# ArmingLou/seed-vc

Measured on AMD Instinct MI355X. Metric: mel_frames_per_sec, higher is better.
Workload: dtype f16; 1 GPU; seed-uvit-tat-xlsr-tiny CFM 25 steps cfg 0.7 + HiFT, batch 64 x (P=430,S=430) per GPU; batch_per_gpu=64, global_batch=64, prompt_frames=430, diffusion_steps=25, vocoder_precision=fp16p8, lanes_per_gpu=2, parallelism=utterance-sharded x1, audio gather on rank 0

## Files before the change

### include/seedvc_hip.h

```cpp
#ifndef SEEDVC_HIP_H
#define SEEDVC_HIP_H

#include <stdint.h>

#ifdef __cplusplus
extern "C" {
#endif

#define SVC_ABI_VERSION 1

typedef struct svc_tensor_desc {
    const char* name;
    const float* data;
    int ndim;
    int64_t shape[4];
} svc_tensor_desc_t;

typedef struct svc_dit_config {
    int version;
    int hidden_dim, num_heads, depth, in_channels, content_dim, style_dim;
    int final_layer_type;
    int time_as_token, style_as_token, uvit_skip_connection, long_skip_connection, style_condition;
    int wn_hidden_dim, wn_num_layers, wn_kernel_size, wn_dilation_rate;
} svc_dit_config_t;

typedef struct svc_dit svc_dit_t;

int svc_dit_create(const svc_dit_config_t* cfg, const svc_tensor_desc_t* weights, int n_weights,
                   void* stream, svc_dit_t** out);
void svc_dit_destroy(svc_dit_t* m);

int svc_dit_set_microbatch(svc_dit_t* m, int utterances);

int svc_dit_set_fused_min_rows(svc_dit_t* m, long rows);
int svc_dit_fused_available(svc_dit_t* m);
int svc_dit_set_graphs(svc_dit_t* m, int on);

typedef struct svc_cfm_args {
    int B;
    int T;
    int P;
    const float* mu;
    const float* prompt;
    const float* style;
    const float* z;
    const int64_t* x_lens;
    const int64_t* prompt_lens;
    int n_timesteps;
    float temperature;
    float cfg_rate[2];
    int random_voice;
    float* out;
} svc_cfm_args_t;

int svc_cfm_sample(svc_dit_t* m, const svc_cfm_args_t* args, void* stream);

int svc_dit_forward(svc_dit_t* m, int N, int T, const float* x, const float* prompt_x, const int64_t* x_lens,
                    float t, const float* style, const float* mu, float* out, void* stream);

typedef struct svc_bigvgan_config {
    int num_mels, upsample_initial_channel, num_upsamples, num_kernels;
    int upsample_rates[8], upsample_kernel_sizes[8];
    int resblock_kernel_sizes[4], resblock_dilation_sizes[4][3];
    int use_tanh_at_final, use_bias_at_final, snake_logscale, snakebeta;
    int precision;
} svc_bigvgan_config_t;
typedef struct svc_bigvgan svc_bigvgan_t;
int svc_bigvgan_create(const svc_bigvgan_config_t* cfg, const svc_tensor_desc_t* weights, int n_weights,
                       void* stream, svc_bigvgan_t** out);
void svc_bigvgan_destroy(svc_bigvgan_t* m);
int svc_bigvgan_forward(svc_bigvgan_t* m, const float* mel, int B, int S, float* out, void* stream);
int svc_bigvgan_forward_ragged(svc_bigvgan_t* m, const float* mel, const int32_t* lens, int B, int S, float* out, void* stream);

typedef struct svc_hift_config {
    int in_channels, base_channels, nb_harmonics, sampling_rate;
    float nsf_alpha, nsf_sigma, nsf_voiced_threshold;
    int num_upsamples, upsample_rates[4], upsample_kernel_sizes[4];
    int istft_n_fft, istft_hop;
    int num_kernels, resblock_kernel_sizes[4], resblock_dilation_sizes[4][3];
    int source_resblock_kernel_sizes[4], source_resblock_dilation_sizes[4][3];
    float lrelu_slope, audio_limit;
    int f0_cond_channels;
    int precision;
} svc_hift_config_t;
typedef struct svc_hift svc_hift_t;
int svc_hift_create(const svc_hift_config_t* cfg, const svc_tensor_desc_t* weights, int n_weights,
                    void* stream, svc_hift_t** out);
void svc_hift_destroy(svc_hift_t* m);
int svc_hift_forward(svc_hift_t* m, const float* mel, const float* f0, const float* phase0, const float* noise,
                     int B, int S, float* out, float* f0_out, void* stream);
int svc_hift_forward_ragged(svc_hift_t* m, const float* mel, const int32_t* lens, const float* f0, const float* phase0,
                            const float* noise, int B, int S, float* out, float* f0_out, void* stream);
int svc_bigvgan_set_microbatch(svc_bigvgan_t* m, int utterances);
int svc_hift_set_microbatch(svc_hift_t* m, int utterances);

typedef struct svc_ar_config {
    int dim, n_head, n_local_heads, head_dim, n_layer, intermediate_size, vocab_size, max_seq_len;
    float rope_base, norm_eps;
} svc_ar_config_t;
typedef struct svc_ar svc_ar_t;
int svc_ar_create(const svc_ar_config_t* cfg, const svc_tensor_desc_t* weights, int n_weights, void* stream, svc_ar_t** out);
void svc_ar_destroy(svc_ar_t* m);
int svc_ar_reset(svc_ar_t* m, void* stream);
int svc_ar_forward_generate(svc_ar_t* m, const float* x, int S, const int64_t* input_pos, const int64_t* kv_pos,
                            float* logits_out, void* stream);
int svc_ar_decode_step(svc_ar_t* m, const float* x, int set_pos, int64_t input_pos, int64_t kv_pos, float* logits_out,
                       void* stream);
int svc_ar_generate(svc_ar_t* m, const float* x_prefill, int S, const int64_t* input_pos, const int64_t* kv_pos,
                    const float* exp_noise, int max_new, int min_tokens_before_eos, float temperature, float top_p,
                    float repetition_penalty, int check_every, int32_t* tokens_out, int32_t* n_tokens, void* stream);
int svc_ar_set_max_batch(svc_ar_t* m, int max_batch, void* stream);
int svc_ar_prefill_slot(svc_ar_t* m, int slot, const float* x, int S, const int64_t* input_pos, const int64_t* kv_pos,
                        float* logits_out, void* stream);
int svc_ar_decode_step_batch(svc_ar_t* m, int B, const float* x, int set_pos, const int64_t* input_pos, const int64_t* kv_pos,
                             float* logits_out, void* stream);
int svc_ar_generate_batch(svc_ar_t* m, int B, const float* x_prefill, const int32_t* S, const int64_t* input_pos,
                          const int64_t* kv_pos, const float* exp_noise, int max_new, int min_tokens_before_eos, float temperature,
                          float top_p, float repetition_penalty, int check_every, int32_t* tokens_out, int32_t* n_tokens,
                          void* stream);
int svc_ar_generate_batch_seeded(svc_ar_t* m, int B, const float* x_prefill, const int32_t* S, const int64_t* input_pos,
                                 const int64_t* kv_pos, const uint64_t* seeds, int max_new, int min_tokens_before_eos,
                                 float temperature, float top_p, float repetition_penalty, int check_every, int32_t* tokens_out,
                                 int32_t* n_tokens, void* stream);
int svc_ar_exp_draws(svc_ar_t* m, uint64_t seed, int step0, int n_steps, float* out, void* stream);
int svc_ar_prefill_batch(svc_ar_t* m, int n, const int32_t* slots, const float* x, const int32_t* S, const int64_t* input_pos,
                         const int64_t* kv_pos, float* logits_out, void* stream);
int svc_ar_set_prefill_rows(svc_ar_t* m, int rows);
int svc_ar_prefill_passes(svc_ar_t* m);
typedef struct svc_ar_request {
    int32_t slot;
    int32_t S;
    const float* exp_noise;
    uint64_t seed;
    int32_t max_new;
    int32_t min_tokens_before_eos;
    float temperature, top_p, repetition_penalty;
    int32_t* tokens_out;
} svc_ar_request_t;
int svc_ar_admit(svc_ar_t* m, int n, const svc_ar_request_t* requests, const float* x_prefill, const int64_t* input_pos,
                 const int64_t* kv_pos, void* stream);
int svc_ar_run(svc_ar_t* m, int n_steps, int32_t* n_tokens, int32_t* done, void* stream);
int svc_ar_retire(svc_ar_t* m, int slot, void* stream);
int svc_ar_session_active(svc_ar_t* m);
int svc_ar_sample(svc_ar_t* m, const float* logits, const int32_t* prev_tokens, int n_prev, int suppress_token,
                  float temperature, float top_p, float repetition_penalty, const float* exp_noise, int32_t* idx_out,
                  float* probs_out, void* stream);

typedef struct svc_lr_config {
    int channels, in_channels, out_channels;
    int is_discrete, codebook_size;
    int n_convs;
    int interpolate;
    int has_final_conv;
    int f0_condition, n_f0_bins;
} svc_lr_config_t;
typedef struct svc_lr svc_lr_t;
int svc_lr_create(const svc_lr_config_t* cfg, const svc_tensor_desc_t* weights, int n_weights, void* stream, svc_lr_t** out);
void svc_lr_destroy(svc_lr_t* m);
int svc_lr_forward(svc_lr_t* m, const float* x, const int64_t* tokens, const int32_t* in_lens, int B, int tin_max,
                   const int32_t* ylens, int tout_max, const float* f0, const int32_t* f0_lens, int tf0_max, float* out,
                   void* stream);

int svc_v2_assemble_cond(const float* prompt_cond, const int32_t* prompt_lens, const float* cond, const int32_t* cond_lens, int B,
                         int Pmax, int Smax, int Dc, int T, float* out, void* stream);
int svc_mel_strip_prompt(const float* mel, const int32_t* prompt_lens, const int32_t* x_lens, int B, int C, int T, int Smax,
                         float pad_value, float* out, void* stream);

int svc_anti_alias_act_fwd(const void* x, void* y, const float* up12, const float* down12,
                           const float* log_alpha, const float* log_beta, int B, int C, int L, int dtype,
                           void* stream);

typedef struct svc_mel svc_mel_t;
int svc_mel_create(int n_fft, int hop, int win, int n_mels, const float* window, const float* mel_basis, void* stream,
                   svc_mel_t** out);
void svc_mel_destroy(svc_mel_t* m);
int svc_mel_frames(const svc_mel_t* m, int L);
int svc_mel_forward(svc_mel_t* m, const float* y, int B, int L, float* out, void* stream);

typedef struct svc_campplus_config {
    int feat_dim, embedding_size, growth_rate, bn_size, init_channels, m_channels;
    int n_blocks, block_layers[4], block_kernel[4], block_dilation[4];
    int seg_len;
} svc_campplus_config_t;
typedef struct svc_campplus svc_campplus_t;
int svc_campplus_create(const svc_campplus_config_t* cfg, const svc_tensor_desc_t* weights, int n_weights, void* stream,
                        svc_campplus_t** out);
void svc_campplus_destroy(svc_campplus_t* m);
int svc_campplus_forward(svc_campplus_t* m, const float* feat, int B, int T, float* out, void* stream);
int svc_kaldi_fbank_frames(int n_samples);
int svc_kaldi_fbank(svc_campplus_t* m, const float* wave, int n_samples, float* out, void* stream);

int svc_crossfade(float* chunk2, const float* chunk1_tail, const double* fade_in, const double* fade_out, int n,
                  void* stream);

int svc_chunks_gather_cond(const float* prompt_cond, const int32_t* prompt_lens, int U, int Pmax, const float* cond, int R,
                           const int32_t* utt, const int32_t* row0, const int32_t* rows, int N, int Dc, int T, float* mu,
                           void* stream);
int svc_chunks_assemble(const float* wave, long long stride, const int32_t* lens, const int32_t* first, const int32_t* last, int N,
                        const double* fade_in, const double* fade_out, int ov, float* out, long long out_len, void* stream);

int svc_sola_step(const float* wave, long long stride, int start, int N, float* sola_state, int max_slots, const int32_t* slots,
                  const float* fade_in, const float* fade_out, int block, int Lb, int Ls, float* out, int32_t* offsets,
                  void* stream);

int svc_op_linear(const float* a, const float* w, const float* bias, float* c, int M, int N, int K, int dtype,
                  int act, void* stream);
int svc_op_conv1d(const float* x, const float* w, const float* bias, float* y, int B, int L, int Cin, int Cout,
                  int k, int dilation, int stride, int pad_left, int Lout, int pad_mode, int dtype, void* stream);
typedef struct {
    const float* x; const uint16_t* a_hi; const uint16_t* a_lo;
    const float* w; const float* bias;
    int32_t B, L, Cin, Cout, k, dilation, pad_left, Lout, dtype;
    const int32_t* seq_len;
    const float* res; const float* res2;
    float out_scale; int32_t act; float act_slope;
    int32_t c_rows, c_off;
    const float* post_a; const float* post_ib; int32_t next_p8;
    int32_t bm, force_gemm;
    float* y; uint16_t* plane_hi; uint16_t* plane_lo;
    int32_t took;
} svc_conv1d_ex_t;
int svc_op_conv1d_ex(svc_conv1d_ex_t* args, void* stream);
int svc_op_conv1d_last_took(void);
int svc_op_conv_transpose1d(const float* x, const float* w, const float* bias, float* y, int B, int L, int Cin,
                            int Cout, int k, int stride, int dtype, void* stream);
int svc_op_attention(const float* q, const float* k, const float* v, float* out, int N, int T, int H,
                     const int64_t* kv_lens_host, void* stream);
int svc_op_rmsnorm(const float* x, const float* gamma, const float* w, const float* b, int add_one, float* y,
                   int rows, int D, void* stream);

int svc_op_gemm_bench(int M, int N, int K, int dtype, int epi, int iters, int debug, float* out_ms, void* stream);
int svc_op_gemm_forms_diff(int M, int N, int K, int epi, int debug_a, int debug_b, long long* n_diff, void* stream);

int svc_prof_enable(int on);
int svc_prof_collect(double* out, int n_cls);

const char* svc_last_error(void);
int svc_abi_version(void);

#ifdef __cplusplus
}
#endif
#endif
```

### seed-vc_amd/_lib.py

```python
import ctypes as C
import os

import torch

_HERE = os.path.dirname(os.path.abspath(__file__))
LIB_PATH = os.path.join(_HERE, "libseedvc_hip.so")

EXPORTS = [
    "svc_abi_version", "svc_last_error",
    "svc_dit_create", "svc_dit_destroy", "svc_dit_set_microbatch", "svc_dit_set_fused_min_rows", "svc_dit_fused_available", "svc_dit_set_graphs", "svc_cfm_sample", "svc_dit_forward",
    "svc_bigvgan_create", "svc_bigvgan_destroy", "svc_bigvgan_forward", "svc_bigvgan_forward_ragged", "svc_bigvgan_set_microbatch",
    "svc_hift_create", "svc_hift_destroy", "svc_hift_forward", "svc_hift_forward_ragged", "svc_hift_set_microbatch",
    "svc_anti_alias_act_fwd",
    "svc_ar_create", "svc_ar_destroy", "svc_ar_reset", "svc_ar_forward_generate", "svc_ar_decode_step", "svc_ar_sample", "svc_ar_generate",
    "svc_ar_set_max_batch", "svc_ar_prefill_slot", "svc_ar_decode_step_batch", "svc_ar_generate_batch",
    "svc_ar_generate_batch_seeded", "svc_ar_exp_draws", "svc_v2_assemble_cond", "svc_mel_strip_prompt",
    "svc_ar_prefill_batch", "svc_ar_set_prefill_rows", "svc_ar_prefill_passes", "svc_ar_admit", "svc_ar_run", "svc_ar_retire",
    "svc_ar_session_active",
    "svc_lr_create", "svc_lr_destroy", "svc_lr_forward", "svc_crossfade",
    "svc_chunks_gather_cond", "svc_chunks_assemble", "svc_sola_step",
    "svc_campplus_create", "svc_campplus_destroy", "svc_campplus_forward", "svc_kaldi_fbank_frames", "svc_kaldi_fbank",
    "svc_mel_create", "svc_mel_destroy", "svc_mel_frames", "svc_mel_forward",
    "svc_prof_enable", "svc_prof_collect",
    "svc_op_linear", "svc_op_conv1d", "svc_op_conv1d_ex", "svc_op_conv1d_last_took", "svc_op_conv_transpose1d", "svc_op_attention", "svc_op_rmsnorm",
]


class TensorDesc(C.Structure):
    _fields_ = [("name", C.c_char_p), ("data", C.c_void_p), ("ndim", C.c_int), ("shape", C.c_int64 * 4)]


class DitConfig(C.Structure):
    _fields_ = [(n, C.c_int) for n in (
        "version", "hidden_dim", "num_heads", "depth", "in_channels", "content_dim", "style_dim",
        "final_layer_type", "time_as_token", "style_as_token", "uvit_skip_connection", "long_skip_connection",
        "style_condition", "wn_hidden_dim", "wn_num_layers", "wn_kernel_size", "wn_dilation_rate")]


class CfmArgs(C.Structure):
    _fields_ = [("B", C.c_int), ("T", C.c_int), ("P", C.c_int),
                ("mu", C.c_void_p), ("prompt", C.c_void_p), ("style", C.c_void_p), ("z", C.c_void_p),
                ("x_lens", C.POINTER(C.c_int64)), ("prompt_lens", C.POINTER(C.c_int64)),
                ("n_timesteps", C.c_int), ("temperature", C.c_float), ("cfg_rate", C.c_float * 2),
                ("random_voice", C.c_int), ("out", C.c_void_p)]


class BigVGANConfig(C.Structure):
    _fields_ = [("num_mels", C.c_int), ("upsample_initial_channel", C.c_int), ("num_upsamples", C.c_int),
                ("num_kernels", C.c_int), ("upsample_rates", C.c_int * 8), ("upsample_kernel_sizes", C.c_int * 8),
                ("resblock_kernel_sizes", C.c_int * 4), ("resblock_dilation_sizes", (C.c_int * 3) * 4),
                ("use_tanh_at_final", C.c_int), ("use_bias_at_final", C.c_int), ("snake_logscale", C.c_int),
                ("snakebeta", C.c_int), ("precision", C.c_int)]


class HiftConfig(C.Structure):
    _fields_ = [("in_channels", C.c_int), ("base_channels", C.c_int), ("nb_harmonics", C.c_int),
                ("sampling_rate", C.c_int), ("nsf_alpha", C.c_float), ("nsf_sigma", C.c_float),
                ("nsf_voiced_threshold", C.c_float), ("num_upsamples", C.c_int), ("upsample_rates", C.c_int * 4),
                ("upsample_kernel_sizes", C.c_int * 4), ("istft_n_fft", C.c_int), ("istft_hop", C.c_int),
                ("num_kernels", C.c_int), ("resblock_kernel_sizes", C.c_int * 4),
                ("resblock_dilation_sizes", (C.c_int * 3) * 4), ("source_resblock_kernel_sizes", C.c_int * 4),
                ("source_resblock_dilation_sizes", (C.c_int * 3) * 4), ("lrelu_slope", C.c_float),
                ("audio_limit", C.c_float), ("f0_cond_channels", C.c_int), ("precision", C.c_int)]


class ArConfig(C.Structure):
    _fields_ = [(n, C.c_int) for n in ("dim", "n_head", "n_local_heads", "head_dim", "n_layer", "intermediate_size",
                                       "vocab_size", "max_seq_len")] + [("rope_base", C.c_float), ("norm_eps", C.c_float)]


class ArRequest(C.Structure):
    _fields_ = [("slot", C.c_int32), ("S", C.c_int32), ("exp_noise", C.c_void_p), ("seed", C.c_uint64), ("max_new", C.c_int32),
                ("min_tokens_before_eos", C.c_int32), ("temperature", C.c_float), ("top_p", C.c_float),
                ("repetition_penalty", C.c_float), ("tokens_out", C.c_void_p)]


class CampplusConfig(C.Structure):
    _fields_ = [(n, C.c_int) for n in ("feat_dim", "embedding_size", "growth_rate", "bn_size", "init_channels", "m_channels", "n_blocks")] + \
               [("block_layers", C.c_int * 4), ("block_kernel", C.c_int * 4), ("block_dilation", C.c_int * 4), ("seg_len", C.c_int)]


class LrConfig(C.Structure):
    _fields_ = [(n, C.c_int) for n in ("channels", "in_channels", "out_channels", "is_discrete", "codebook_size", "n_convs",
                                       "interpolate", "has_final_conv", "f0_condition", "n_f0_bins")]


class Conv1dEx(C.Structure):
    _fields_ = [("x", C.c_void_p), ("a_hi", C.c_void_p), ("a_lo", C.c_void_p), ("w", C.c_void_p), ("bias", C.c_void_p)] + \
               [(n, C.c_int32) for n in ("B", "L", "Cin", "Cout", "k", "dilation", "pad_left", "Lout", "dtype")] + \
               [("seq_len", C.POINTER(C.c_int32)), ("res", C.c_void_p), ("res2", C.c_void_p),
                ("out_scale", C.c_float), ("act", C.c_int32), ("act_slope", C.c_float), ("c_rows", C.c_int32), ("c_off", C.c_int32),
                ("post_a", C.c_void_p), ("post_ib", C.c_void_p), ("next_p8", C.c_int32), ("bm", C.c_int32), ("force_gemm", C.c_int32),
                ("y", C.c_void_p), ("plane_hi", C.c_void_p), ("plane_lo", C.c_void_p), ("took", C.c_int32)]


_lib = None


def lib():
    global _lib
    if _lib is None:
        if not os.path.exists(LIB_PATH):
            raise ImportError(f"{LIB_PATH} is missing: run `python -c 'import __graft_entry__ as g; g.build()'` "
                              f"(hipcc --offload-arch=gfx950); there is no CPU fallback")
        l = C.CDLL(LIB_PATH)
        l.svc_last_error.restype = C.c_char_p
        if l.svc_abi_version() != 1:
            raise ImportError("libseedvc_hip.so ABI version mismatch")
        l.svc_sola_step.argtypes = [C.c_void_p, C.c_longlong, C.c_int, C.c_int, C.c_void_p, C.c_int, C.POINTER(C.c_int32),
                                    C.c_void_p, C.c_void_p, C.c_int, C.c_int, C.c_int, C.c_void_p, C.c_void_p, C.c_void_p]
        l.svc_hift_forward_ragged.argtypes = [C.c_void_p, C.c_void_p, C.POINTER(C.c_int32), C.c_void_p, C.c_void_p, C.c_void_p,
                                              C.c_int, C.c_int, C.c_void_p, C.c_void_p, C.c_void_p]
        l.svc_op_conv1d_ex.argtypes = [C.POINTER(Conv1dEx), C.c_void_p]
        _lib = l
    return _lib


def check(rc):
    if rc != 0:
        raise RuntimeError("seedvc_hip: " + (lib().svc_last_error() or b"unknown error").decode())


def stream_ptr():
    return C.c_void_p(torch.cuda.current_stream().cuda_stream)


def ptr(t):
    return C.c_void_p(t.data_ptr()) if t is not None else C.c_void_p(0)


def f32c(t, device=None):
    t = t.detach()
    if device is not None:
        t = t.to(device)
    return t.to(torch.float32).contiguous()


def make_descs(state_dict, device):
    keep, items = [], []
    for k, v in state_dict.items():
        if not torch.is_tensor(v) or not (v.is_floating_point()):
            continue
        if v.dim() > 4:
            continue
        t = f32c(v, device)
        keep.append(t)
        items.append((k, t))
    arr = (TensorDesc * len(items))()
    for i, (k, t) in enumerate(items):
        kb = k.encode()
        keep.append(kb)
        arr[i].name = kb
        arr[i].data = t.data_ptr()
        arr[i].ndim = t.dim()
        for j in range(4):
            arr[i].shape[j] = t.shape[j] if j < t.dim() else 1
    return arr, len(items), keep


def i64_host(values):
    if values is None:
        return None
    vals = [int(v) for v in values]
    return (C.c_int64 * len(vals))(*vals)
```

### seed-vc_amd/cfm.py

```python
import ctypes as C

import torch

from . import _lib
from .specs import dit_config


def _cfg_struct(cfg):
    c = _lib.DitConfig()
    c.version = cfg["version"]
    c.hidden_dim, c.num_heads, c.depth = cfg["D"], cfg["H"], cfg["L"]
    c.in_channels, c.content_dim, c.style_dim = cfg["C"], cfg["Dc"], cfg["style_dim"]
    c.final_layer_type = 1 if cfg["head"] == "wavenet" else 0
    c.time_as_token, c.style_as_token = int(cfg["time_as_token"]), int(cfg["style_as_token"])
    c.uvit_skip_connection, c.long_skip_connection = int(cfg["uvit"]), int(cfg["long_skip"])
    c.style_condition = int(cfg["style_condition"])
    c.wn_hidden_dim = cfg.get("wn_dim", 0)
    c.wn_num_layers = cfg.get("wn_layers", 0)
    c.wn_kernel_size = cfg.get("wn_kernel", 0)
    c.wn_dilation_rate = cfg.get("wn_dilation", 1)
    return c


class Estimator:

    def __init__(self, cfg, state_dict, device="cuda:0"):
        self.cfg = cfg
        self.device = torch.device(device)
        self.in_channels = cfg["C"]
        self._h = C.c_void_p()
        with torch.cuda.device(self.device):
            descs, n, keep = _lib.make_descs(state_dict, self.device)
            cs = _cfg_struct(cfg)
            _lib.check(_lib.lib().svc_dit_create(C.byref(cs), descs, n, _lib.stream_ptr(), C.byref(self._h)))
            torch.cuda.current_stream().synchronize()
        del keep

    def setup_caches(self, max_batch_size=1, max_seq_length=8192):
        return None

    def set_microbatch(self, n):
        _lib.check(_lib.lib().svc_dit_set_microbatch(self._h, int(n)))

    def set_fused_min_rows(self, rows):
        _lib.check(_lib.lib().svc_dit_set_fused_min_rows(self._h, C.c_long(int(rows))))

    def set_graphs(self, on):
        _lib.check(_lib.lib().svc_dit_set_graphs(self._h, int(bool(on))))

    @property
    def fused_available(self):
        return bool(_lib.lib().svc_dit_fused_available(self._h))

    def __call__(self, x, prompt_x, x_lens, t, style, cond, mask_content=False):
        N, Cc, T = x.shape
        with torch.cuda.device(self.device):
            x, prompt_x, style, cond = (_lib.f32c(a, self.device) for a in (x, prompt_x, style, cond))
            out = torch.empty_like(x)
            tval = float(t.reshape(-1)[0]) if torch.is_tensor(t) else float(t)
            lens = None
            if x_lens is not None:
                xl = [int(v) for v in (x_lens.tolist() if torch.is_tensor(x_lens) else x_lens)]
                if len(xl) == 1 and N > 1:
                    xl = xl * N
                lens = _lib.i64_host(xl)
            _lib.check(_lib.lib().svc_dit_forward(self._h, N, T, _lib.ptr(x), _lib.ptr(prompt_x), lens,
                                                  C.c_float(tval), _lib.ptr(style), _lib.ptr(cond), _lib.ptr(out),
                                                  _lib.stream_ptr()))
        return out

    def close(self):
        if self._h:
            _lib.lib().svc_dit_destroy(self._h)
            self._h = C.c_void_p()

    def __del__(self):
        try:
            self.close()
        except Exception:
            pass


class CFM:

    def __init__(self, cfg, state_dict, device="cuda:0"):
        self.cfg = cfg
        self.estimator = Estimator(cfg, state_dict, device)
        self.in_channels = cfg["C"]
        self.device = self.estimator.device

    @classmethod
    def from_preset(cls, name, state_dict, device="cuda:0", **overrides):
        return cls(dit_config(name, **overrides), state_dict, device)

    @torch.inference_mode()
    def inference(self, mu, x_lens, prompt, style, f0=None, n_timesteps=10, temperature=1.0,
                  inference_cfg_rate=0.5, random_voice=False, z=None, prompt_lens=None):
        if self.cfg["version"] == 2 and not isinstance(f0, (type(None), torch.Tensor)):
            n_timesteps, f0 = f0, None
        B, T = mu.size(0), mu.size(1)
        dev = self.device
        with torch.cuda.device(dev):
            mu, prompt, style = (_lib.f32c(a, dev) for a in (mu, prompt, style))
            if z is None:
                z = torch.randn([B, self.in_channels, T], device=dev)
            z = _lib.f32c(z, dev)
            out = torch.empty(B, self.in_channels, T, device=dev, dtype=torch.float32)
            a = _lib.CfmArgs()
            a.B, a.T, a.P = B, T, prompt.size(-1)
            a.mu, a.prompt, a.style, a.z, a.out = (t.data_ptr() for t in (mu, prompt, style, z, out))
            xl = None
            if x_lens is not None:
                xl = [int(v) for v in (x_lens.tolist() if torch.is_tensor(x_lens) else x_lens)]
                if len(xl) == 1 and B > 1:
                    xl = xl * B
            lens_keep = _lib.i64_host(xl)
            plens_keep = _lib.i64_host(prompt_lens)
            a.x_lens = lens_keep
            a.prompt_lens = plens_keep
            a.n_timesteps = int(n_timesteps)
            a.temperature = float(temperature)
            if isinstance(inference_cfg_rate, (list, tuple)):
                a.cfg_rate[0], a.cfg_rate[1] = float(inference_cfg_rate[0]), float(inference_cfg_rate[1])
            else:
                a.cfg_rate[0], a.cfg_rate[1] = float(inference_cfg_rate), float(inference_cfg_rate)
            a.random_voice = int(bool(random_voice))
            _lib.check(_lib.lib().svc_cfm_sample(self.estimator._h, C.byref(a), _lib.stream_ptr()))
        return out
```

### seed-vc_amd/csrc/common.h

```cpp
#pragma once
#include <atomic>
#include <hip/hip_runtime.h>
#include <stdint.h>
#include <stdio.h>
#include <string>

namespace svc {

typedef _Float16 half_t;
typedef _Float16 half8 __attribute__((ext_vector_type(8)));
typedef _Float16 half4 __attribute__((ext_vector_type(4)));
typedef _Float16 half2v __attribute__((ext_vector_type(2)));
typedef float float4v __attribute__((ext_vector_type(4)));
typedef unsigned int u32x4 __attribute__((ext_vector_type(4)));

void set_error(const std::string& msg);
const char* get_error();

#define SVC_CHECK_HIP(expr)                                                                  \
    do {                                                                                     \
        hipError_t _e = (expr);                                                              \
        if (_e != hipSuccess) {                                                              \
            svc::set_error(std::string(#expr) + ": " + hipGetErrorString(_e) + " at " + __FILE__ + \
                           ":" + std::to_string(__LINE__));                                  \
            return 1;                                                                        \
        }                                                                                    \
    } while (0)

#define SVC_REQUIRE(cond, msg)                                                               \
    do {                                                                                     \
        if (!(cond)) {                                                                       \
            svc::set_error(std::string("requirement failed: ") + #cond + " -- " + (msg));    \
            return 1;                                                                        \
        }                                                                                    \
    } while (0)

__device__ __forceinline__ float sin_sq(float x) {
    const float n = rintf(x * 0.318309886183790672f);
    float r = fmaf(n, -3.140625f, x);
    r = fmaf(n, -9.67502593994140625e-4f, r);
    r = fmaf(n, -1.509957990978376e-7f, r);
    const float r2 = r * r;
    float p = fmaf(r2, 2.6348154733568663e-06f, -0.00019822761532850564f);
    p = fmaf(p, r2, 0.008333242498338223f);
    p = fmaf(p, r2, -0.1666666567325592f);
    const float sn = fmaf(p * r2, r, r);
    return sn * sn;
}

struct DeviceState {
    int device = -1;
    void* zero_page = nullptr;
    std::atomic<unsigned long long> kconv_attr{0};
    std::atomic<bool> fused_attr{false};
};
DeviceState* device_state();
int current_device();

enum { PROF_KGEMM_F16 = 0, PROF_KGEMM_F32 = 1, PROF_ATTN = 2, PROF_FUSED = 3, PROF_N = 4 };
bool prof_enabled();
void prof_begin(int cls, hipStream_t st);
void prof_end(int cls, double flops, double bytes, hipStream_t st, unsigned long long tag = 0);

template <int MAXA, int DPT>
__device__ __forceinline__ void wait_tiles(int ahead) {
    static_assert(MAXA * DPT <= 63, "vmcnt is a 6-bit counter");
    if constexpr (MAXA <= 0) {
        asm volatile("s_waitcnt vmcnt(0)" ::: "memory");
    } else {
        if (ahead >= MAXA) asm volatile("s_waitcnt vmcnt(%0)" ::"n"(MAXA * DPT) : "memory");
        else wait_tiles<MAXA - 1, DPT>(ahead);
    }
}

__device__ __forceinline__ float act_apply(float v, int act, float slope);
__device__ __forceinline__ uint4 pack8(const float* v) {
    half8 h;
#pragma unroll
    for (int j = 0; j < 8; ++j) h[j] = (half_t)v[j];
    return *reinterpret_cast<uint4*>(&h);
}

static inline int cdiv(long a, long b) { return (int)((a + b - 1) / b); }
static inline long round_up(long a, long b) { return (a + b - 1) / b * b; }

constexpr int KG_MAX_TAPS = 48;

enum { KG_PAD_ZERO = 0, KG_PAD_REFLECT = 1, KG_PAD_CLAMP = 2 };
enum { KG_ACT_NONE = 0, KG_ACT_SILU = 1, KG_ACT_ELU = 2, KG_ACT_LRELU = 3, KG_ACT_TANH = 4, KG_ACT_ABS = 5,
       KG_ACT_CLAMP = 6 , KG_ACT_SIGMOID = 7 };
enum {
    KG_EPI_STORE = 0,
    KG_EPI_SWIGLU = 1,
    KG_EPI_TANHSIG = 2,
    KG_EPI_QKV_ROPE = 3,
};

__device__ __forceinline__ float act_apply(float v, int act, float slope) {
    switch (act) {
        case KG_ACT_SILU: return v / (1.0f + __expf(-v));
        case KG_ACT_ELU: return v > 0.f ? v : (expm1f(v));
        case KG_ACT_LRELU: return v > 0.f ? v : v * slope;
        case KG_ACT_TANH: return tanhf(v);
        case KG_ACT_ABS: return fabsf(v);
        case KG_ACT_CLAMP: return fminf(fmaxf(v, -slope), slope);
        case KG_ACT_SIGMOID: return 1.0f / (1.0f + __expf(-v));
        default: return v;
    }
}

struct KGemmParams {
    const void* a_ptr[KG_MAX_TAPS];
    long a_ld[KG_MAX_TAPS];
    int a_shift[KG_MAX_TAPS];
    int a_ktiles[KG_MAX_TAPS];
    int n_taps;
    int Lout, a_seq_rows, a_off, a_stride, a_len, pad_mode;
    int reflect_min;
    const int* seq_len;
    const void* zero_page;
    float prof_flop_scale;
    int debug;
    int group_n;
    const void* w;
    long ldw;
    int M, N;
    int c_seq_rows, c_off;
    float* c32; long ldc32;
    half_t* c16; long ldc16;
    const float* post_a; const float* post_ib; int post_n; half_t* c16_lo;
    const float* bias;
    const float* rowvec; long ld_rowvec;
    const float* gate;   long ld_gate;
    const float* res;    long ldres;
    const float* res2;   long ldres2;
    float out_scale;
    int act; float act_slope;
    int post_relu;
    int vec_ok;
    const float* rope;
    int rope_D;
    float q_scale;
    half_t* vt; long vt_seq_stride; long vt_ld;
    int vt_mode;
};

int kgemm_launch(const KGemmParams& p, int dtype , int epi, hipStream_t st);
int kgemm_big_launch(const KGemmParams& p, int epi, hipStream_t st);

struct KConvParams {
    const void* a_hi; const void* a_lo;
    const void* w; long ldw;
    const float* bias;
    int B, Lin, Lout, N, cin_pad, k, dil, pad_left, nsub;
    int c_seq_rows, c_off;
    float* c32; long ldc32;
    half_t* c16; half_t* c16_lo; long ldc16;
    const float* post_a; const float* post_ib; int post_n;
    const float* res; long ldres;
    const float* res2; long ldres2;
    float out_scale;
    int act; float act_slope;
    const void* zero_page;
    int w8_exp;
    int c16_lo_fmt;
    const int* seq_len;
    int bm;
    int* took;
};
bool kconv_enabled();
int kconv_launch(const KConvParams& p, hipStream_t st);
__device__ __forceinline__ unsigned lo_pair_p8(float hi_as_float, float lo) {
    const float a = __builtin_amdgcn_fmed3f(hi_as_float, -448.f, 448.f), b = __builtin_amdgcn_fmed3f(lo * 2048.f, -448.f, 448.f);
    return (unsigned)__builtin_amdgcn_cvt_pk_fp8_f32(a, b, 0, false) & 0xffffu;
}
int kconv_pack_p8(const float* src, unsigned short* dst, int n0, int n1, int n2, long s0, long s1, long s2, long d0, long d1, long d2,
                  const float* scale, int* exp_out, hipStream_t st);

struct PanelParams {
    int M;
    int Lout, seq_rows, row_off;
    const half_t* wstream;
    int n_slots;
    float eps;
    int do_post;
    const half_t* ao;
    float* x;
    const float* gate_a; const float* gate_f;
    const float* g_ffn; const float* w_f; const float* b_f; int add_one;
    int I;
    half_t* c16;
    int do_skip;
    const half_t* skip_in; const float* bskip;
    int do_qkv;
    const float* g_attn; const float* w_a; const float* b_a;
    const float* rope; float q_scale;
    half_t* qk; half_t* vt; long vt_seq_stride; long vt_ld; int vt_mode;
    int do_final;
    const float* g_fin; const float* w_fin; const float* b_fin; half_t* n16;
};
bool fused_supported(int D, int I);
long fused_stream_halfs(int D, int I, bool post, bool skip, bool qkv);
long fused_pack_stream(half_t* dst, int D, int I, const float* wo, const float* w1, const float* w3, const float* w2,
                       const float* wskip, const float* wqkv, hipStream_t st);
int fused_panel_launch(const PanelParams& p, int D, bool gated, hipStream_t st);

struct AttnParams {
    const half_t* q; const half_t* k; long ld_qk;
    const half_t* vt; long vt_seq_stride; long vt_ld;
    half_t* out; long ld_out;
    int n_seq, H, seq_rows, Tq;
    int q_start;
    const int* kv_len; int kv_len_const;
    int vt_perm;
};
__host__ __device__ inline int vt_perm_pos(int pos) {
    return (pos & ~31) | (((pos >> 2) & 3) << 3) | (((pos >> 4) & 1) << 2) | (pos & 3);
}
__host__ __device__ inline int vt_perm_pos16(int pos) {
    return (pos & ~12) | ((pos & 4) << 1) | ((pos & 8) >> 1);
}
__host__ __device__ inline int vt_pos(int pos, int mode) {
    return mode == 2 ? vt_perm_pos16(pos) : (mode == 1 ? vt_perm_pos(pos) : pos);
}
int attention_vt_mode(int n_seq, int H, int Tq);
int attention_launch(const AttnParams& p, hipStream_t st);
int attention_permute_vt(half_t* vt, long rows, long vt_ld, int mode, hipStream_t st);

int rmsnorm_mod_launch(const float* x, long ldx, half_t* y, long ldy, const float* gamma,
                       const float* w, const float* b, long ld_wb, int add_one,
                       int rows, int D, int seq_rows, float eps, hipStream_t st);
int layernorm_mod_launch(const float* x, long ldx, half_t* y, long ldy, const float* scale,
                         const float* shift, int rows, int D, float eps, hipStream_t st);

}
```

### seed-vc_amd/csrc/device.hip

```cpp
#include <map>
#include <mutex>

#include "common.h"

namespace svc {

int current_device() {
    int d = -1;
    if (hipGetDevice(&d) != hipSuccess) return -1;
    return d;
}

DeviceState* device_state() {
    static std::mutex mu;
    static std::map<int, DeviceState*> states;
    const int d = current_device();
    if (d < 0) {
        set_error("hipGetDevice failed");
        return nullptr;
    }
    std::lock_guard<std::mutex> lk(mu);
    auto it = states.find(d);
    if (it != states.end()) return it->second;
    void* zp = nullptr;
    if (hipMalloc(&zp, 256) != hipSuccess || hipMemset(zp, 0, 256) != hipSuccess) {
        set_error("device_state: zero page allocation failed");
        return nullptr;
    }
    DeviceState* s = new DeviceState();
    s->device = d;
    s->zero_page = zp;
    states[d] = s;
    return s;
}

}
```

### seed-vc_amd/csrc/dit.hip

```cpp
#include <math.h>
#include <string.h>

#include <algorithm>
#include <vector>

#include "model_util.h"

using namespace svc;

namespace {
constexpr int MAX_STREAMS = 3;
constexpr int ROPE_POS = 8192;

float bf16_round(float f) {
    uint32_t u;
    memcpy(&u, &f, 4);
    u = (u + 0x7FFF + ((u >> 16) & 1)) & 0xFFFF0000u;
    memcpy(&f, &u, 4);
    return f;
}

std::vector<float> linspace01(int n) {
    std::vector<float> v(n);
    const float step = 1.0f / (float)(n - 1);
    const int half = n / 2;
    for (int i = 0; i < n; ++i) v[i] = i < half ? 0.0f + step * (float)i : 1.0f - step * (float)(n - 1 - i);
    return v;
}
}

struct svc_dit {
    svc_dit_config_t cfg;
    int D, H, L, C, Dc, S, I, W, NL, WK, npre, C16, C32;
    bool v2, wavenet, adaptive_blocks;
    Arena wts, ws;
    struct StepGraph {
        std::vector<float> key;
        hipGraphExec_t exec = nullptr;
        int seen = 0;
    };
    std::vector<StepGraph> graphs;
    hipStream_t cap_stream = nullptr;
    int use_graphs = 0;
    void drop_graphs() {
        for (auto& g : graphs) if (g.exec) (void)hipGraphExecDestroy(g.exec);
        graphs.clear();
    }
    PinnedRing staging;
    hipStream_t create_stream;
    int device = -1;

    struct Layer {
        half_t *wqkv, *wo, *w13, *w2, *wskip;
        float *bskip, *g_attn, *g_ffn;
        half_t* stream = nullptr;
        int stream_slots = 0;
    };
    half_t* stream_pre = nullptr;
    int stream_pre_slots = 0;
    bool fused_ok = false;
    long fused_min_rows = 10240;
    std::vector<Layer> layers;
    float* g_final;
    std::vector<int> emit, recv;
    float *te_w0, *te_b0, *te_w2, *te_b2, *te_freqs;
    float *te2_w0, *te2_b0, *te2_w2, *te2_b2, *te2_freqs;
    float *mod_w, *mod_b;
    int mod_n;
    int mod_layer_n;
    half_t* w_merge_x;
    float* w_stat;
    float* stat_const;
    float* w_style_merge;
    float *style_in_w, *style_in_b;
    half_t *head_wa, *head_w2;
    float *head_b0, *head_b2;
    half_t *w_longskip, *w_conv1, *w_resproj, *w_fl, *w_conv2;
    float *b_longskip, *b_conv1, *b_resproj, *b_fl, *b_conv2;
    float *wn_cond_w, *wn_cond_b, *fl_mod_w, *fl_mod_b;
    std::vector<half_t*> wn_in, wn_res, wn_skip;
    std::vector<float*> wn_res_b, wn_skip_b;
    half_t* wn_tail = nullptr;
    float* b_tail = nullptr;
    long acts_stride = 0;
    float* rope;

    int cap_streams = 0, cap_B = 0, cap_T = 0, cap_steps = 0;
    int seq_rows = 0, vt_ld = 0;
    float *x32, *xin, *st_term, *v32, *u_rowvec, *tok_style, *prompt32, *wnx32, *flin32;
    half_t *x16, *n16, *qk16, *vt, *ao16, *ff16, *h16, *hm16, *xr16, *wnx16, *acts16, *fl16, *fo16;
    std::vector<half_t*> skip16;
    int *d_kvlen, *d_convlen, *d_plen;
    int* d_convlen_w = nullptr;
    int win0 = 0;
    float *d_tvals, *d_tfeat, *d_th, *d_t1, *d_t1s, *d_t2, *d_mod, *d_gcond, *d_flmod, *d_stylevec;
    int microbatch = 0;

    int pack(const StateDict& sd, hipStream_t st);
    int reserve(int n_streams, int B, int T, int n_steps, hipStream_t st);
    int tables(const std::vector<float>& tvals, hipStream_t st);
    int statics(int n_streams, const int (*flags)[3], int B, int T, const float* mu, const float* style_dev,
                hipStream_t st);
    int run_group(const svc_cfm_args_t* a, int b0, int nb, int n_streams, const int (*flags)[3],
                  const std::vector<float>& tvals, const std::vector<float>& dts, float c0, float ca, float cb,
                  int stream_a, int stream_b, hipStream_t st);
    int body(int n_streams, int B, int T, int step, hipStream_t st);
    int body_fused(int n_streams, int B, int T, int step, hipStream_t st);
    int head(int n_streams, int B, int T, int step, hipStream_t st);
};

namespace {

int pack_block(int dtype, const float* src, long src_ld, long src_col, int N, int K, void* dst, long ldw, long dst_col,
               long dst_row0, long dst_row_step, const float* scale, hipStream_t st) {
    return pack_any(dtype, src + src_col, dst, dst_row0 * ldw + dst_col, N, 1, K, src_ld, 0, 1, dst_row_step * ldw, 0, 1,
                    scale, st);
}

float* copy_vec(Arena& ar, const float* src, long n, hipStream_t st) {
    float* d = ar.alloc_n<float>(n, st);
    if (!d) return nullptr;
    if (hipMemcpyAsync(d, src, n * sizeof(float), hipMemcpyDeviceToDevice, st) != hipSuccess) {
        set_error("hipMemcpyAsync failed");
        return nullptr;
    }
    return d;
}

}

#define GETW(var, name, ...)                                              \
    const svc_tensor_desc_t* var = sd.get(name);                          \
    if (require_shape(var, name, {__VA_ARGS__})) return 1;

int svc_dit::pack(const StateDict& sd, hipStream_t st) {
    const long Dp = round_up(D, 128);
    auto new16 = [&](long rows, long ld) { return wts.alloc_n<half_t>(round_up(rows, 128) * ld, st); };
    layers.resize(L);
    for (int i = 0; i < L; ++i) {
        const std::string p = "transformer.layers." + std::to_string(i) + ".";
        Layer& ly = layers[i];
        GETW(wqkv, p + "attention.wqkv.weight", 3 * D, D);
        GETW(wo, p + "attention.wo.weight", D, D);
        GETW(w1, p + "feed_forward.w1.weight", I, D);
        GETW(w3, p + "feed_forward.w3.weight", I, D);
        GETW(w2, p + "feed_forward.w2.weight", D, I);
        ly.wqkv = new16(3 * D, D);
        ly.wo = new16(D, D);
        ly.w13 = new16(2 * I, D);
        ly.w2 = new16(D, I);
        if (!ly.wqkv || !ly.wo || !ly.w13 || !ly.w2) return 1;
        if (pack_block(0, wqkv->data, D, 0, 3 * D, D, ly.wqkv, D, 0, 0, 1, nullptr, st)) return 1;
        if (pack_block(0, wo->data, D, 0, D, D, ly.wo, D, 0, 0, 1, nullptr, st)) return 1;
        if (pack_block(0, w1->data, D, 0, I, D, ly.w13, D, 0, 0, 2, nullptr, st)) return 1;
        if (pack_block(0, w3->data, D, 0, I, D, ly.w13, D, 0, 1, 2, nullptr, st)) return 1;
        if (pack_block(0, w2->data, I, 0, D, I, ly.w2, I, 0, 0, 1, nullptr, st)) return 1;
        const std::string an = v2 ? p + "attention_norm.norm.weight" : p + "attention_norm.norm.weight";
        const std::string fn = v2 ? p + "ffn_norm.weight" : p + "ffn_norm.norm.weight";
        GETW(ga, an, D);
        GETW(gf, fn, D);
        ly.g_attn = copy_vec(wts, ga->data, D, st);
        ly.g_ffn = copy_vec(wts, gf->data, D, st);
        if (!ly.g_attn || !ly.g_ffn) return 1;
        ly.wskip = nullptr;
        ly.bskip = nullptr;
        if (std::find(recv.begin(), recv.end(), i) != recv.end()) {
            GETW(ws_, p + "skip_in_linear.weight", D, 2 * D);
            GETW(bs_, p + "skip_in_linear.bias", D);
            ly.wskip = new16(D, 2 * D);
            if (!ly.wskip) return 1;
            if (pack_block(0, ws_->data, 2 * D, 0, D, 2 * D, ly.wskip, 2 * D, 0, 0, 1, nullptr, st)) return 1;
            ly.bskip = copy_vec(wts, bs_->data, D, st);
            if (!ly.bskip) return 1;
        }
    }
    {
        GETW(gn, "transformer.norm.norm.weight", D);
        g_final = copy_vec(wts, gn->data, D, st);
        if (!g_final) return 1;
    }
    fused_ok = fused_supported(D, I);
    if (fused_ok) {
        auto W = [&](const std::string& k) { return sd.get(k)->data; };
        const int slot_halfs = (D / 16) * 512;
        for (int i = 0; i < L; ++i) {
            const std::string p = "transformer.layers." + std::to_string(i) + ".";
            const bool last = i == L - 1;
            const bool nskip = !last && layers[i + 1].wskip != nullptr;
            const std::string pn = "transformer.layers." + std::to_string(i + 1) + ".";
            const long halfs = fused_stream_halfs(D, I, true, nskip, !last);
            layers[i].stream = wts.alloc_n<half_t>(halfs, st);
            if (!layers[i].stream) return 1;
            const long wr = fused_pack_stream(layers[i].stream, D, I, W(p + "attention.wo.weight"), W(p + "feed_forward.w1.weight"),
                                              W(p + "feed_forward.w3.weight"), W(p + "feed_forward.w2.weight"),
                                              nskip ? W(pn + "skip_in_linear.weight") : nullptr,
                                              last ? nullptr : W(pn + "attention.wqkv.weight"), st);
            if (wr != halfs) { set_error("fused stream packing failed"); return 1; }
            layers[i].stream_slots = (int)(halfs / slot_halfs);
        }
        const long halfs = fused_stream_halfs(D, I, false, false, true);
        stream_pre = wts.alloc_n<half_t>(halfs, st);
        if (!stream_pre) return 1;
        if (fused_pack_stream(stream_pre, D, I, nullptr, nullptr, nullptr, nullptr, nullptr,
                              W("transformer.layers.0.attention.wqkv.weight"), st) != halfs) { set_error("fused stream packing failed"); return 1; }
        stream_pre_slots = (int)(halfs / slot_halfs);
    }
    mod_layer_n = adaptive_blocks ? (v2 ? 6 * D : 4 * D) : 0;
    mod_n = L * mod_layer_n + 2 * D;
    mod_w = wts.alloc_n<float>((long)mod_n * D, st);
    mod_b = wts.alloc_n<float>(mod_n, st);
    if (!mod_w || !mod_b) return 1;
    auto put_mod = [&](const std::string& wname, const std::string& bname, int rows, long row0) -> int {
        GETW(w, wname, rows, D);
        GETW(b, bname, rows);
        if (pack_f32_launch(w->data, mod_w + row0 * D, rows, 1, D, D, 0, 1, D, 0, 1, nullptr, st)) return 1;
        SVC_CHECK_HIP(hipMemcpyAsync(mod_b + row0, b->data, rows * sizeof(float), hipMemcpyDeviceToDevice, st));
        return 0;
    };
    for (int i = 0; i < L && adaptive_blocks; ++i) {
        const std::string p = "transformer.layers." + std::to_string(i) + ".";
        if (v2) {
            if (put_mod(p + "attention_norm.linear.weight", p + "attention_norm.linear.bias", 6 * D, (long)i * mod_layer_n)) return 1;
        } else {
            if (put_mod(p + "attention_norm.project_layer.weight", p + "attention_norm.project_layer.bias", 2 * D, (long)i * mod_layer_n)) return 1;
            if (put_mod(p + "ffn_norm.project_layer.weight", p + "ffn_norm.project_layer.bias", 2 * D, (long)i * mod_layer_n + 2 * D)) return 1;
        }
    }
    if (v2) {
        if (put_mod("transformer.norm.linear.weight", "transformer.norm.linear.bias", 2 * D, (long)L * mod_layer_n)) return 1;
    } else {
        if (put_mod("transformer.norm.project_layer.weight", "transformer.norm.project_layer.bias", 2 * D, (long)L * mod_layer_n)) return 1;
    }
    auto put_temb = [&](const std::string& p, int dim, float** w0, float** b0, float** w2, float** b2, float** fr) -> int {
        GETW(a, p + ".mlp.0.weight", dim, 256);
        GETW(b, p + ".mlp.0.bias", dim);
        GETW(c, p + ".mlp.2.weight", dim, dim);
        GETW(d, p + ".mlp.2.bias", dim);
        *w0 = copy_vec(wts, a->data, (long)dim * 256, st);
        *b0 = copy_vec(wts, b->data, dim, st);
        *w2 = copy_vec(wts, c->data, (long)dim * dim, st);
        *b2 = copy_vec(wts, d->data, dim, st);
        if (!*w0 || !*b0 || !*w2 || !*b2) return 1;
        if (const auto* f = sd.get(p + ".freqs")) {
            if (require_shape(f, p + ".freqs", {128})) return 1;
            *fr = copy_vec(wts, f->data, 128, st);
        } else {
            std::vector<float> h(128);
            for (int i = 0; i < 128; ++i) h[i] = expf(-logf(10000.0f) * (float)i / 128.0f);
            *fr = wts.alloc_n<float>(128, st);
            if (*fr) SVC_CHECK_HIP(hipMemcpyAsync(*fr, h.data(), 512, hipMemcpyHostToDevice, st));
            SVC_CHECK_HIP(hipStreamSynchronize(st));
        }
        return *fr ? 0 : 1;
    };
    if (put_temb("t_embedder", D, &te_w0, &te_b0, &te_w2, &te_b2, &te_freqs)) return 1;

    const bool style_in_merge = !v2 && cfg.style_condition && !cfg.style_as_token;
    const int Kin = D + 2 * C + (style_in_merge ? S : 0);
    GETW(wm, "cond_x_merge_linear.weight", D, Kin);
    GETW(bm, "cond_x_merge_linear.bias", D);
    GETW(wcp, "cond_projection.weight", D, Dc);
    GETW(bcp, "cond_projection.bias", D);
    w_merge_x = new16(D, C16);
    if (!w_merge_x) return 1;
    if (pack_block(0, wm->data, Kin, 0, D, C, w_merge_x, C16, 0, 0, 1, nullptr, st)) return 1;
    const long Ks = C32 + Dc;
    w_stat = wts.alloc_n<float>(Dp * Ks, st);
    stat_const = wts.alloc_n<float>(D, st);
    if (!w_stat || !stat_const) return 1;
    if (pack_block(1, wm->data, Kin, C, D, C, w_stat, Ks, 0, 0, 1, nullptr, st)) return 1;
    {
        float* wcpT = ws.alloc_n<float>((long)Dc * D, st);
        if (!wcpT) return 1;
        if (pack_f32_launch(wcp->data, wcpT, D, 1, Dc, Dc, 0, 1, 1, 0, D, nullptr, st)) return 1;
        if (small_linear_launch(wm->data + 2 * C, Kin, wcpT, D, nullptr, w_stat + C32, Ks, D, Dc, D, KG_ACT_NONE, st)) return 1;
        if (small_linear_launch(bcp->data, D, wm->data + 2 * C, Kin, bm->data, stat_const, D, 1, D, D, KG_ACT_NONE, st)) return 1;
    }
    w_style_merge = nullptr;
    if (style_in_merge) {
        w_style_merge = wts.alloc_n<float>((long)D * S, st);
        if (!w_style_merge) return 1;
        if (pack_f32_launch(wm->data + 2 * C + D, w_style_merge, D, 1, S, Kin, 0, 1, S, 0, 1, nullptr, st)) return 1;
    }
    style_in_w = style_in_b = nullptr;
    if (v2 || cfg.style_as_token) {
        GETW(sw, "style_in.weight", D, S);
        GETW(sb, "style_in.bias", D);
        style_in_w = copy_vec(wts, sw->data, (long)D * S, st);
        style_in_b = copy_vec(wts, sb->data, D, st);
        if (!style_in_w || !style_in_b) return 1;
    }
    if (!wavenet) {
        GETW(a, "final_mlp.0.weight", D, D);
        GETW(b, "final_mlp.0.bias", D);
        GETW(c, "final_mlp.2.weight", C, D);
        GETW(d, "final_mlp.2.bias", C);
        head_wa = new16(D, D);
        head_w2 = new16(C, D);
        if (!head_wa || !head_w2) return 1;
        if (pack_block(0, a->data, D, 0, D, D, head_wa, D, 0, 0, 1, nullptr, st)) return 1;
        if (pack_block(0, c->data, D, 0, C, D, head_w2, D, 0, 0, 1, nullptr, st)) return 1;
        head_b0 = copy_vec(wts, b->data, D, st);
        head_b2 = copy_vec(wts, d->data, C, st);
        if (!head_b0 || !head_b2) return 1;
    } else {
        if (put_temb("t_embedder2", W, &te2_w0, &te2_b0, &te2_w2, &te2_b2, &te2_freqs)) return 1;
        if (cfg.long_skip_connection) {
            GETW(a, "skip_linear.weight", D, D + C);
            GETW(b, "skip_linear.bias", D);
            w_longskip = new16(D, D + C16);
            if (!w_longskip) return 1;
            if (pack_block(0, a->data, D + C, 0, D, D + C, w_longskip, D + C16, 0, 0, 1, nullptr, st)) return 1;
            b_longskip = copy_vec(wts, b->data, D, st);
            if (!b_longskip) return 1;
        }
        GETW(c1w, "conv1.weight", W, D);
        GETW(c1b, "conv1.bias", W);
        GETW(rpw, "res_projection.weight", W, D);
        GETW(rpb, "res_projection.bias", W);
        GETW(c2w, "conv2.weight", C, W, 1);
        GETW(c2b, "conv2.bias", C);
        w_conv1 = new16(W, D);
        w_resproj = new16(W, D);
        w_conv2 = new16(C, W);
        if (!w_conv1 || !w_resproj || !w_conv2) return 1;
        if (pack_block(0, c1w->data, D, 0, W, D, w_conv1, D, 0, 0, 1, nullptr, st)) return 1;
        if (pack_block(0, rpw->data, D, 0, W, D, w_resproj, D, 0, 0, 1, nullptr, st)) return 1;
        if (pack_block(0, c2w->data, W, 0, C, W, w_conv2, W, 0, 0, 1, nullptr, st)) return 1;
        b_conv1 = copy_vec(wts, c1b->data, W, st);
        b_resproj = copy_vec(wts, rpb->data, W, st);
        b_conv2 = copy_vec(wts, c2b->data, C, st);
        if (!b_conv1 || !b_resproj || !b_conv2) return 1;
        {
            WeightSrc fl;
            if (resolve_weight(sd, "final_layer.linear", wts, st, &fl)) return 1;
            if (require_shape(fl.desc, "final_layer.linear.weight", {W, W})) return 1;
            GETW(flb, "final_layer.linear.bias", W);
            GETW(mw, "final_layer.adaLN_modulation.1.weight", 2 * W, W);
            GETW(mb, "final_layer.adaLN_modulation.1.bias", 2 * W);
            w_fl = new16(W, W);
            if (!w_fl) return 1;
            if (pack_block(0, fl.v, W, 0, W, W, w_fl, W, 0, 0, 1, fl.scale, st)) return 1;
            b_fl = copy_vec(wts, flb->data, W, st);
            fl_mod_w = copy_vec(wts, mw->data, 2L * W * W, st);
            fl_mod_b = copy_vec(wts, mb->data, 2 * W, st);
            if (!b_fl || !fl_mod_w || !fl_mod_b) return 1;
        }
        {
            WeightSrc cl;
            if (resolve_weight(sd, "wavenet.cond_layer.conv.conv", wts, st, &cl)) return 1;
            if (require_shape(cl.desc, "wavenet.cond_layer.conv.conv.weight", {2L * W * NL, W, 1})) return 1;
            GETW(clb, "wavenet.cond_layer.conv.conv.bias", 2L * W * NL);
            wn_cond_w = wts.alloc_n<float>(2L * W * NL * W, st);
            wn_cond_b = wts.alloc_n<float>(2L * W * NL, st);
            float* tmp_b = ws.alloc_n<float>(2L * W * NL, st);
            if (!wn_cond_w || !wn_cond_b || !tmp_b) return 1;
            wn_in.resize(NL);
            wn_res.assign(NL, nullptr);
            wn_skip.resize(NL);
            wn_res_b.assign(NL, nullptr);
            wn_skip_b.resize(NL);
            for (int i = 0; i < NL; ++i) {
                const std::string li = std::to_string(i);
                for (int half = 0; half < 2; ++half) {
                    const long src_row0 = 2L * W * i + (long)half * W;
                    if (pack_f32_launch(cl.v + src_row0 * W, wn_cond_w + (2L * W * i + half) * W, W, 1, W, W, 0, 1, 2L * W, 0, 1,
                                        cl.scale ? cl.scale + src_row0 : nullptr, st)) return 1;
                    if (pack_f32_launch(clb->data + src_row0, tmp_b + 2L * W * i + half, W, 1, 1, 1, 0, 0, 2, 0, 0, nullptr, st)) return 1;
                }
                WeightSrc in;
                if (resolve_weight(sd, "wavenet.in_layers." + li + ".conv.conv", wts, st, &in)) return 1;
                if (require_shape(in.desc, "wavenet.in_layers." + li + ".conv.conv.weight", {2L * W, W, WK})) return 1;
                GETW(inb, "wavenet.in_layers." + li + ".conv.conv.bias", 2L * W);
                wn_in[i] = new16(2 * W, (long)WK * W);
                float* inb_perm = ws.alloc_n<float>(2L * W, st);
                if (!wn_in[i] || !inb_perm) return 1;
                for (int half = 0; half < 2; ++half) {
                    if (pack_f16_launch(in.v + (long)half * W * W * WK, wn_in[i] + (long)half * WK * W, W, WK, W,
                                        (long)W * WK, 1, WK, 2L * WK * W, W, 1, in.scale ? in.scale + (long)half * W : nullptr, st)) return 1;
                    if (pack_f32_launch(inb->data + (long)half * W, inb_perm + half, W, 1, 1, 1, 0, 0, 2, 0, 0, nullptr, st)) return 1;
                }
                {
                    float* dst = wn_cond_b + 2L * W * i;
                    if (add_rowvec_launch(dst, tmp_b + 2L * W * i, 0, inb_perm, 1, 2 * W, st)) return 1;
                }
                WeightSrc rs;
                const int rs_out = i < NL - 1 ? 2 * W : W;
                if (resolve_weight(sd, "wavenet.res_skip_layers." + li + ".conv.conv", wts, st, &rs)) return 1;
                if (require_shape(rs.desc, "wavenet.res_skip_layers." + li + ".conv.conv.weight", {rs_out, W, 1})) return 1;
                GETW(rsb, "wavenet.res_skip_layers." + li + ".conv.conv.bias", rs_out);
                const long skip_row0 = i < NL - 1 ? W : 0;
                if (i < NL - 1) {
                    wn_res[i] = new16(W, W);
                    if (!wn_res[i]) return 1;
                    if (pack_block(0, rs.v, W, 0, W, W, wn_res[i], W, 0, 0, 1, rs.scale, st)) return 1;
                    wn_res_b[i] = copy_vec(wts, rsb->data, W, st);
                    if (!wn_res_b[i]) return 1;
                }
                wn_skip[i] = new16(W, W);
                if (!wn_skip[i]) return 1;
                if (pack_block(0, rs.v + skip_row0 * W, W, 0, W, W, wn_skip[i], W, 0, 0, 1,
                               rs.scale ? rs.scale + skip_row0 : nullptr, st)) return 1;
                wn_skip_b[i] = copy_vec(wts, rsb->data + skip_row0, W, st);
                if (!wn_skip_b[i]) return 1;
            }
        }
    }
    if (wavenet) {
        const long Kt = (long)NL * W + D;
        wn_tail = new16(W, Kt);
        b_tail = wts.alloc_n<float>(W, st);
        if (!wn_tail || !b_tail) return 1;
        for (int i = 0; i < NL; ++i)
            SVC_CHECK_HIP(hipMemcpy2DAsync(wn_tail + (long)i * W, Kt * 2, wn_skip[i], (size_t)W * 2, (size_t)W * 2, W, hipMemcpyDeviceToDevice, st));
        SVC_CHECK_HIP(hipMemcpy2DAsync(wn_tail + (long)NL * W, Kt * 2, w_resproj, (size_t)D * 2, (size_t)D * 2, W, hipMemcpyDeviceToDevice, st));
        if (add_rowvec_launch(b_tail, b_resproj, 0, wn_skip_b[0], 1, W, st)) return 1;
        for (int i = 1; i < NL; ++i)
            if (add_rowvec_launch(b_tail, b_tail, 0, wn_skip_b[i], 1, W, st)) return 1;
    }
    {
        std::vector<float> tab((size_t)ROPE_POS * 32 * 2);
        for (int i = 0; i < 32; ++i) {
            const float e = (float)(2 * i) / 64.0f;
            const float f = 1.0f / powf(10000.0f, e);
            for (int t = 0; t < ROPE_POS; ++t) {
                const float a = (float)t * f;
                float c = (float)cos((double)a), s = (float)sin((double)a);
                if (v2) { c = bf16_round(c); s = bf16_round(s); }
                tab[((size_t)t * 32 + i) * 2] = c;
                tab[((size_t)t * 32 + i) * 2 + 1] = s;
            }
        }
        rope = wts.alloc_n<float>(tab.size(), st);
        if (!rope) return 1;
        SVC_CHECK_HIP(hipMemcpyAsync(rope, tab.data(), tab.size() * 4, hipMemcpyHostToDevice, st));
        SVC_CHECK_HIP(hipStreamSynchronize(st));
    }
    SVC_CHECK_HIP(hipStreamSynchronize(st));
    ws.release();
    return 0;
}

int svc_dit::reserve(int n_streams, int B, int T, int n_steps, hipStream_t st) {
    if (n_streams <= cap_streams && B <= cap_B && T <= cap_T && n_steps <= cap_steps) {
        seq_rows = (int)round_up(T + npre, 8);
        vt_ld = (int)round_up(seq_rows, 64);
        return 0;
    }
    SVC_CHECK_HIP(hipStreamSynchronize(st));
    drop_graphs();
    ws.release();
    cap_streams = std::max(cap_streams, n_streams);
    cap_B = std::max(cap_B, B);
    cap_T = std::max(cap_T, T);
    cap_steps = std::max(cap_steps, n_steps);
    const long rows_seq = round_up(cap_T + npre, 8);
    const long nseq = (long)cap_streams * cap_B;
    const long M = nseq * rows_seq;
    const long vtl = round_up(rows_seq, 64);
    x32 = ws.alloc_n<float>((long)cap_B * rows_seq * C16, st);
    x16 = ws.alloc_n<half_t>(M * C16, st);
    xin = ws.alloc_n<float>(M * D, st);
    st_term = ws.alloc_n<float>(M * D, st);
    v32 = ws.alloc_n<float>(M * C16, st);
    u_rowvec = ws.alloc_n<float>(nseq * D, st);
    tok_style = ws.alloc_n<float>(nseq * D, st);
    prompt32 = ws.alloc_n<float>((long)cap_B * rows_seq * C32, st);
    n16 = ws.alloc_n<half_t>(M * D, st);
    qk16 = ws.alloc_n<half_t>(M * 2 * D, st);
    vt = ws.alloc_n<half_t>(nseq * D * vtl, st);
    ao16 = ws.alloc_n<half_t>(M * D, st);
    ff16 = ws.alloc_n<half_t>(M * I, st);
    h16 = ws.alloc_n<half_t>(M * D, st);
    skip16.assign(emit.size(), nullptr);
    for (auto& p : skip16) {
        p = ws.alloc_n<half_t>(M * D, st);
        if (!p) return 1;
    }
    if (!x32 || !x16 || !xin || !st_term || !v32 || !u_rowvec || !tok_style || !prompt32 || !n16 || !qk16 || !vt ||
        !ao16 || !ff16 || !h16)
        return 1;
    hm16 = xr16 = wnx16 = acts16 = fl16 = fo16 = nullptr;
    wnx32 = flin32 = nullptr;
    if (!wavenet) {
        hm16 = ws.alloc_n<half_t>(M * D, st);
        if (!hm16) return 1;
    } else {
        xr16 = ws.alloc_n<half_t>(M * D, st);
        wnx32 = ws.alloc_n<float>(M * W, st);
        wnx16 = ws.alloc_n<half_t>(M * W, st);
        acts_stride = M * W;
        acts16 = ws.alloc_n<half_t>((long)NL * acts_stride, st);
        flin32 = ws.alloc_n<float>(M * W, st);
        fl16 = ws.alloc_n<half_t>(M * W, st);
        fo16 = ws.alloc_n<half_t>(M * W, st);
        if (!xr16 || !wnx32 || !wnx16 || !acts16 || !flin32 || !fl16 || !fo16) return 1;
    }
    d_kvlen = ws.alloc_n<int>(nseq, st);
    d_convlen = ws.alloc_n<int>(nseq, st);
    d_convlen_w = ws.alloc_n<int>(nseq, st);
    d_plen = ws.alloc_n<int>(cap_B, st);
    const long Sx = cap_steps;
    d_tvals = ws.alloc_n<float>(Sx, st);
    d_tfeat = ws.alloc_n<float>(Sx * 256, st);
    d_th = ws.alloc_n<float>(Sx * std::max(D, W), st);
    d_t1 = ws.alloc_n<float>(Sx * D, st);
    d_t1s = ws.alloc_n<float>(Sx * D, st);
    d_t2 = ws.alloc_n<float>(Sx * std::max(W, 1), st);
    d_mod = ws.alloc_n<float>(Sx * mod_n, st);
    d_gcond = ws.alloc_n<float>(Sx * std::max(2L * W * NL, 1L), st);
    d_flmod = ws.alloc_n<float>(Sx * std::max(2 * W, 1), st);
    d_stylevec = ws.alloc_n<float>((long)cap_B * D, st);
    if (!d_kvlen || !d_convlen || !d_convlen_w || !d_plen || !d_tvals || !d_tfeat || !d_th || !d_t1 || !d_t1s || !d_t2 || !d_mod ||
        !d_gcond || !d_flmod || !d_stylevec)
        return 1;
    seq_rows = (int)round_up(T + npre, 8);
    vt_ld = (int)round_up(seq_rows, 64);
    SVC_CHECK_HIP(hipStreamSynchronize(st));
    return 0;
}

int svc_dit::tables(const std::vector<float>& tvals, hipStream_t st) {
    const int n = (int)tvals.size();
    {
        float* h = reinterpret_cast<float*>(staging.acquire(n * sizeof(float)));
        if (!h) return 1;
        memcpy(h, tvals.data(), n * sizeof(float));
        SVC_CHECK_HIP(hipMemcpyAsync(d_tvals, h, n * sizeof(float), hipMemcpyHostToDevice, st));
        if (staging.commit(st)) return 1;
    }
    if (timestep_feat_launch(d_tvals, te_freqs, d_tfeat, n, st)) return 1;
    if (small_linear_launch(d_tfeat, 256, te_w0, 256, te_b0, d_th, D, n, D, 256, KG_ACT_SILU, st)) return 1;
    if (small_linear_launch(d_th, D, te_w2, D, te_b2, d_t1, D, n, D, D, KG_ACT_NONE, st)) return 1;
    if (silu_launch(d_t1, d_t1s, (long)n * D, st)) return 1;
    if (small_linear_launch(v2 ? d_t1s : d_t1, D, mod_w, D, mod_b, d_mod, mod_n, n, mod_n, D, KG_ACT_NONE, st)) return 1;
    if (wavenet) {
        if (small_linear_launch(d_tfeat, 256, te2_w0, 256, te2_b0, d_th, W, n, W, 256, KG_ACT_SILU, st)) return 1;
        if (small_linear_launch(d_th, W, te2_w2, W, te2_b2, d_t2, W, n, W, W, KG_ACT_NONE, st)) return 1;
        if (small_linear_launch(d_t2, W, wn_cond_w, W, wn_cond_b, d_gcond, 2L * W * NL, n, 2 * W * NL, W, KG_ACT_NONE, st)) return 1;
        if (small_linear_launch(d_t1s, D, fl_mod_w, W, fl_mod_b, d_flmod, 2 * W, n, 2 * W, W, KG_ACT_NONE, st)) return 1;
    }
    return 0;
}


namespace {
KGemmParams gemm_base(int M, int N, int Lout) {
    KGemmParams p;
    memset(&p, 0, sizeof(p));
    p.M = M;
    p.N = N;
    p.Lout = Lout;
    p.a_seq_rows = Lout;
    p.c_seq_rows = Lout;
    p.a_stride = 1;
    p.a_len = Lout;
    p.n_taps = 1;
    p.vec_ok = 1;
    return p;
}
}

int svc_dit::body(int n_streams, int B, int T, int step, hipStream_t st) {
    const int nseq = n_streams * B;
    const int M = nseq * seq_rows;
    const float* mod = d_mod + (long)step * mod_n;
    if (prefix_rows_launch(xin, nseq, seq_rows, D, npre, T + npre, d_t1 + (long)step * D, tok_style,
                           cfg.time_as_token ? 1 : 0, st)) return 1;
    {
        KGemmParams p = gemm_base(nseq * T, D, T);
        p.a_ptr[0] = x16; p.a_ld[0] = C16; p.a_ktiles[0] = C16 / 64;
        p.a_seq_rows = seq_rows; p.a_len = T;
        p.w = w_merge_x; p.ldw = C16;
        p.c_seq_rows = seq_rows; p.c_off = npre;
        p.c32 = xin; p.ldc32 = D;
        p.res = st_term; p.ldres = D;
        if (kgemm_launch(p, 0, KG_EPI_STORE, st)) return 1;
    }
    if (fused_ok && (long)M >= fused_min_rows) {
        if (body_fused(n_streams, B, T, step, st)) return 1;
        return head(n_streams, B, T, step, st);
    }
    const int Lw = seq_rows - win0;
    auto gemm_win = [&](int N) {
        KGemmParams p = gemm_base(nseq * Lw, N, Lw);
        p.a_seq_rows = seq_rows; p.c_seq_rows = seq_rows;
        p.a_off = win0; p.c_off = win0;
        return p;
    };
    size_t emit_i = 0;
    std::vector<int> skip_stack;
    for (int i = 0; i < L; ++i) {
        const bool tail_only = i == L - 1 && win0 > 0;

        const Layer& ly = layers[i];
        const float* lmod = adaptive_blocks ? mod + (long)i * mod_layer_n : nullptr;
        const bool is_recv = ly.wskip != nullptr;
        if (is_recv) {
            const int src = skip_stack.back();
            skip_stack.pop_back();
            KGemmParams p = gemm_base(M, D, seq_rows);
            p.n_taps = 2;
            p.a_ptr[0] = h16; p.a_ld[0] = D; p.a_ktiles[0] = D / 64;
            p.a_ptr[1] = skip16[src]; p.a_ld[1] = D; p.a_ktiles[1] = D / 64;
            p.w = ly.wskip; p.ldw = 2 * D;
            p.bias = ly.bskip;
            p.c32 = xin; p.ldc32 = D;
            if (kgemm_launch(p, 0, KG_EPI_STORE, st)) return 1;
        }
        const float *w_a = nullptr, *b_a = nullptr, *gate_a = nullptr, *w_f = nullptr, *b_f = nullptr, *gate_f = nullptr;
        if (lmod) {
            if (v2) {
                b_a = lmod; w_a = lmod + D; gate_a = lmod + 2 * D;
                b_f = lmod + 3 * D; w_f = lmod + 4 * D; gate_f = lmod + 5 * D;
            } else {
                w_a = lmod; b_a = lmod + D; w_f = lmod + 2 * D; b_f = lmod + 3 * D;
            }
        }
        if (rmsnorm_mod_launch(xin, D, n16, D, ly.g_attn, w_a, b_a, 0, v2 ? 1 : 0, M, D, seq_rows, 1e-5f, st)) return 1;
        {
            KGemmParams p = gemm_base(M, 3 * D, seq_rows);
            p.a_ptr[0] = n16; p.a_ld[0] = D; p.a_ktiles[0] = D / 64;
            p.w = ly.wqkv; p.ldw = D;
            p.c16 = qk16; p.ldc16 = 2 * D;
            p.rope = rope; p.rope_D = D; p.q_scale = 0.125f * 1.4426950408889634f;
            p.vt = vt; p.vt_seq_stride = (long)D * vt_ld; p.vt_ld = vt_ld; p.vt_mode = attention_vt_mode(nseq, H, seq_rows);
            if (kgemm_launch(p, 0, KG_EPI_QKV_ROPE, st)) return 1;
        }
        {
            AttnParams a;
            memset(&a, 0, sizeof(a));
            a.q = qk16; a.k = qk16 + D; a.ld_qk = 2 * D;
            a.vt = vt; a.vt_seq_stride = (long)D * vt_ld; a.vt_ld = vt_ld; a.vt_perm = attention_vt_mode(nseq, H, seq_rows);
            a.out = ao16; a.ld_out = D;
            a.n_seq = nseq; a.H = H; a.seq_rows = seq_rows; a.Tq = seq_rows;
            a.q_start = tail_only ? win0 : 0;
            a.kv_len = d_kvlen;
            if (attention_launch(a, st)) return 1;
        }
        {
            KGemmParams p = tail_only ? gemm_win(D) : gemm_base(M, D, seq_rows);
            p.a_ptr[0] = ao16; p.a_ld[0] = D; p.a_ktiles[0] = D / 64;
            p.w = ly.wo; p.ldw = D;
            p.gate = gate_a; p.ld_gate = 0;
            p.res = xin; p.ldres = D;
            p.c32 = xin; p.ldc32 = D;
            if (kgemm_launch(p, 0, KG_EPI_STORE, st)) return 1;
        }
        if (rmsnorm_mod_launch(xin, D, n16, D, ly.g_ffn, w_f, b_f, 0, v2 ? 1 : 0, M, D, seq_rows, 1e-5f, st)) return 1;
        {
            KGemmParams p = tail_only ? gemm_win(2 * I) : gemm_base(M, 2 * I, seq_rows);
            p.a_ptr[0] = n16; p.a_ld[0] = D; p.a_ktiles[0] = D / 64;
            p.w = ly.w13; p.ldw = D;
            p.c16 = ff16; p.ldc16 = I;
            if (kgemm_launch(p, 0, KG_EPI_SWIGLU, st)) return 1;
        }
        {
            KGemmParams p = tail_only ? gemm_win(D) : gemm_base(M, D, seq_rows);
            p.a_ptr[0] = ff16; p.a_ld[0] = I; p.a_ktiles[0] = I / 64;
            p.w = ly.w2; p.ldw = I;
            p.gate = gate_f; p.ld_gate = 0;
            p.res = xin; p.ldres = D;
            p.c32 = xin; p.ldc32 = D;
            const bool is_emit = std::find(emit.begin(), emit.end(), i) != emit.end();
            const bool next_recv = i + 1 < L && layers[i + 1].wskip != nullptr;
            if (is_emit) {
                p.c16 = skip16[emit_i]; p.ldc16 = D;
                skip_stack.push_back((int)emit_i);
                ++emit_i;
            } else if (next_recv) {
                p.c16 = h16; p.ldc16 = D;
            }
            if (kgemm_launch(p, 0, KG_EPI_STORE, st)) return 1;
        }
    }
    {
        const float* fm = mod + (long)L * mod_layer_n;
        const float* w = fm;
        const float* b = fm + D;
        if (rmsnorm_mod_launch(xin, D, n16, D, g_final, w, b, 0, v2 ? 1 : 0, M, D, seq_rows, 1e-5f, st)) return 1;
    }
    return head(n_streams, B, T, step, st);
}

int svc_dit::head(int n_streams, int B, int T, int step, hipStream_t st) {
    const int nseq = n_streams * B;
    const int M = nseq * seq_rows;
    const int Lw = seq_rows - win0;
    auto gemm_win = [&](int N) {
        KGemmParams p = gemm_base(nseq * Lw, N, Lw);
        p.a_seq_rows = seq_rows; p.c_seq_rows = seq_rows;
        p.a_off = win0; p.c_off = win0;
        return p;
    };
    if (!wavenet) {
        {
            KGemmParams p = gemm_win(D);
            p.a_ptr[0] = n16; p.a_ld[0] = D; p.a_ktiles[0] = D / 64;
            p.w = head_wa; p.ldw = D; p.bias = head_b0; p.act = KG_ACT_SILU;
            p.c16 = hm16; p.ldc16 = D;
            if (kgemm_launch(p, 0, KG_EPI_STORE, st)) return 1;
        }
        {
            KGemmParams p = gemm_win(C);
            p.a_ptr[0] = hm16; p.a_ld[0] = D; p.a_ktiles[0] = D / 64;
            p.w = head_w2; p.ldw = D; p.bias = head_b2;
            p.c32 = v32; p.ldc32 = C16;
            if (kgemm_launch(p, 0, KG_EPI_STORE, st)) return 1;
        }
        return 0;
    }
    const half_t* xres16 = n16;
    if (cfg.long_skip_connection) {
        KGemmParams p = gemm_win(D);
        p.n_taps = 2;
        p.a_ptr[0] = n16; p.a_ld[0] = D; p.a_ktiles[0] = D / 64;
        p.a_ptr[1] = x16; p.a_ld[1] = C16; p.a_ktiles[1] = C16 / 64;
        p.w = w_longskip; p.ldw = D + C16; p.bias = b_longskip;
        p.c16 = xr16; p.ldc16 = D;
        if (kgemm_launch(p, 0, KG_EPI_STORE, st)) return 1;
        xres16 = xr16;
    }
    {
        KGemmParams p = gemm_win(W);
        p.a_ptr[0] = xres16; p.a_ld[0] = D; p.a_ktiles[0] = D / 64;
        p.w = w_conv1; p.ldw = D; p.bias = b_conv1;
        p.c32 = wnx32; p.ldc32 = W; p.c16 = wnx16; p.ldc16 = W;
        if (kgemm_launch(p, 0, KG_EPI_STORE, st)) return 1;
    }
    for (int i = 0; i < NL; ++i) {
        int dil = 1;
        for (int j = 0; j < i; ++j) dil *= cfg.wn_dilation_rate;
        {
            KGemmParams p = gemm_win(2 * W);
            p.n_taps = WK;
            const int total = (WK - 1) * dil;
            const int left = total - total / 2;
            for (int t = 0; t < WK; ++t) {
                p.a_ptr[t] = wnx16; p.a_ld[t] = W; p.a_ktiles[t] = W / 64; p.a_shift[t] = t * dil - left;
            }
            p.pad_mode = KG_PAD_REFLECT;
            p.reflect_min = std::max(left, total - left) + 1;
            p.seq_len = d_convlen_w;
            p.w = wn_in[i]; p.ldw = (long)WK * W;
            p.rowvec = d_gcond + (long)step * 2 * W * NL + 2L * W * i; p.ld_rowvec = 0;
            p.c16 = acts16 + (long)i * acts_stride; p.ldc16 = W;
            if (kgemm_launch(p, 0, KG_EPI_TANHSIG, st)) return 1;
        }
        if (i < NL - 1) {
            KGemmParams p = gemm_win(W);
            p.a_ptr[0] = acts16 + (long)i * acts_stride; p.a_ld[0] = W; p.a_ktiles[0] = W / 64;
            p.w = wn_res[i]; p.ldw = W; p.bias = wn_res_b[i];
            p.res = wnx32; p.ldres = W;
            p.c32 = wnx32; p.ldc32 = W; p.c16 = wnx16; p.ldc16 = W;
            if (kgemm_launch(p, 0, KG_EPI_STORE, st)) return 1;
        }
    }
    {
        KGemmParams p = gemm_win(W);
        p.n_taps = NL + 1;
        for (int i = 0; i < NL; ++i) {
            p.a_ptr[i] = acts16 + (long)i * acts_stride; p.a_ld[i] = W; p.a_ktiles[i] = W / 64;
        }
        p.a_ptr[NL] = xres16; p.a_ld[NL] = D; p.a_ktiles[NL] = D / 64;
        p.w = wn_tail; p.ldw = (long)NL * W + D; p.bias = b_tail;
        p.c32 = flin32; p.ldc32 = W;
        if (kgemm_launch(p, 0, KG_EPI_STORE, st)) return 1;
    }
    {
        const float* fm = d_flmod + (long)step * 2 * W;
        if (layernorm_mod_launch(flin32, W, fl16, W, fm + W, fm, M, W, 1e-6f, st)) return 1;
    }
    {
        KGemmParams p = gemm_win(W);
        p.a_ptr[0] = fl16; p.a_ld[0] = W; p.a_ktiles[0] = W / 64;
        p.w = w_fl; p.ldw = W; p.bias = b_fl;
        p.c16 = fo16; p.ldc16 = W;
        if (kgemm_launch(p, 0, KG_EPI_STORE, st)) return 1;
    }
    {
        KGemmParams p = gemm_win(C);
        p.a_ptr[0] = fo16; p.a_ld[0] = W; p.a_ktiles[0] = W / 64;
        p.w = w_conv2; p.ldw = W; p.bias = b_conv2;
        p.c32 = v32; p.ldc32 = C16;
        if (kgemm_launch(p, 0, KG_EPI_STORE, st)) return 1;
    }
    return 0;
}

int svc_dit::body_fused(int n_streams, int B, int T, int step, hipStream_t st) {
    const int nseq = n_streams * B;
    const int M = nseq * seq_rows;
    const float* mod = d_mod + (long)step * mod_n;
    auto mods = [&](int i, const float** w_a, const float** b_a, const float** gate_a, const float** w_f, const float** b_f,
                    const float** gate_f) {
        *w_a = *b_a = *gate_a = *w_f = *b_f = *gate_f = nullptr;
        if (!adaptive_blocks) return;
        const float* lmod = mod + (long)i * mod_layer_n;
        if (v2) {
            *b_a = lmod; *w_a = lmod + D; *gate_a = lmod + 2 * D;
            *b_f = lmod + 3 * D; *w_f = lmod + 4 * D; *gate_f = lmod + 5 * D;
        } else {
            *w_a = lmod; *b_a = lmod + D; *w_f = lmod + 2 * D; *b_f = lmod + 3 * D;
        }
    };
    auto base = [&]() {
        PanelParams p;
        memset(&p, 0, sizeof(p));
        p.M = M; p.Lout = seq_rows; p.seq_rows = seq_rows; p.row_off = 0;
        p.eps = 1e-5f; p.add_one = v2 ? 1 : 0; p.I = I; p.x = xin;
        return p;
    };
    auto set_qkv = [&](PanelParams& p, int layer) {
        const float *w_a, *b_a, *ga, *w_f, *b_f, *gf;
        mods(layer, &w_a, &b_a, &ga, &w_f, &b_f, &gf);
        p.do_qkv = 1;
        p.g_attn = layers[layer].g_attn; p.w_a = w_a; p.b_a = b_a;
        p.rope = rope; p.q_scale = 0.125f * 1.4426950408889634f;
        p.qk = qk16; p.vt = vt; p.vt_seq_stride = (long)D * vt_ld; p.vt_ld = vt_ld; p.vt_mode = attention_vt_mode(nseq, H, seq_rows);
    };
    {
        PanelParams p = base();
        p.wstream = stream_pre; p.n_slots = stream_pre_slots;
        set_qkv(p, 0);
        if (fused_panel_launch(p, D, v2, st)) return 1;
    }
    size_t emit_i = 0;
    std::vector<int> skip_stack;
    for (int i = 0; i < L; ++i) {
        const bool last = i == L - 1;
        const bool tail_only = last && win0 > 0;
        {
            AttnParams a;
            memset(&a, 0, sizeof(a));
            a.q = qk16; a.k = qk16 + D; a.ld_qk = 2 * D;
            a.vt = vt; a.vt_seq_stride = (long)D * vt_ld; a.vt_ld = vt_ld; a.vt_perm = attention_vt_mode(nseq, H, seq_rows);
            a.out = ao16; a.ld_out = D;
            a.n_seq = nseq; a.H = H; a.seq_rows = seq_rows; a.Tq = seq_rows;
            a.q_start = tail_only ? win0 : 0;
            a.kv_len = d_kvlen;
            if (attention_launch(a, st)) return 1;
        }
        PanelParams p = base();
        const float *w_a, *b_a, *ga, *w_f, *b_f, *gf;
        mods(i, &w_a, &b_a, &ga, &w_f, &b_f, &gf);
        p.wstream = layers[i].stream; p.n_slots = layers[i].stream_slots;
        p.do_post = 1; p.ao = ao16;
        p.gate_a = ga; p.gate_f = gf; p.g_ffn = layers[i].g_ffn; p.w_f = w_f; p.b_f = b_f;
        if (std::find(emit.begin(), emit.end(), i) != emit.end()) {
            p.c16 = skip16[emit_i];
            skip_stack.push_back((int)emit_i);
            ++emit_i;
        }
        if (!last) {
            if (layers[i + 1].wskip) {
                p.do_skip = 1;
                p.skip_in = skip16[skip_stack.back()];
                skip_stack.pop_back();
                p.bskip = layers[i + 1].bskip;
            }
            set_qkv(p, i + 1);
        } else {
            const float* fm = mod + (long)L * mod_layer_n;
            p.do_final = 1; p.g_fin = g_final; p.w_fin = fm; p.b_fin = fm + D; p.n16 = n16;
            if (tail_only) { p.Lout = seq_rows - win0; p.row_off = win0; p.M = nseq * p.Lout; }
        }
        if (fused_panel_launch(p, D, v2, st)) return 1;
    }
    return 0;
}

int svc_dit::statics(int n_streams, const int (*flags)[3], int B, int T, const float* mu, const float* style_dev,
                     hipStream_t st) {
    const long Ks = C32 + Dc;
    if (w_style_merge)
        if (small_linear_launch(style_dev, S, w_style_merge, S, nullptr, d_stylevec, D, B, D, S, KG_ACT_NONE, st)) return 1;
    for (int j = 0; j < n_streams; ++j) {
        const bool use_p = flags[j][0], use_s = flags[j][1], use_m = flags[j][2];
        float* u = u_rowvec + (long)j * B * D;
        if (add_rowvec_launch(u, (use_s && w_style_merge) ? d_stylevec : nullptr, D, stat_const, B, D, st)) return 1;
        float* dst = st_term + (long)j * B * seq_rows * D;
        {
            KGemmParams p = gemm_base(B * T, D, T);
            p.a_ptr[0] = mu; p.a_ld[0] = Dc; p.a_ktiles[0] = use_m ? Dc / 32 : 0;
            p.a_seq_rows = T; p.a_len = T;
            p.w = w_stat + C32; p.ldw = Ks;
            p.c_seq_rows = seq_rows; p.c_off = npre;
            p.c32 = dst; p.ldc32 = D;
            p.rowvec = u; p.ld_rowvec = D;
            if (kgemm_launch(p, 1, KG_EPI_STORE, st)) return 1;
        }
        if (use_p) {
            KGemmParams p = gemm_base(B * T, D, T);
            p.a_ptr[0] = prompt32; p.a_ld[0] = C32; p.a_ktiles[0] = C32 / 32;
            p.a_seq_rows = seq_rows; p.a_len = T;
            p.w = w_stat; p.ldw = Ks;
            p.c_seq_rows = seq_rows; p.c_off = npre;
            p.c32 = dst; p.ldc32 = D;
            p.res = dst; p.ldres = D;
            if (kgemm_launch(p, 1, KG_EPI_STORE, st)) return 1;
        }
        if (style_in_w) {
            float* tk = tok_style + (long)j * B * D;
            if (use_s) {
                if (small_linear_launch(style_dev, S, style_in_w, S, style_in_b, tk, D, B, D, S, KG_ACT_NONE, st)) return 1;
            } else {
                if (add_rowvec_launch(tk, nullptr, 0, style_in_b, B, D, st)) return 1;
            }
        }
    }
    return 0;
}

namespace {
__global__ void init_state_kernel(float* __restrict__ x, long ldx, half_t* __restrict__ x16, long ldx16, int rows, int B,
                                  int T, int C, const int* __restrict__ prompt_len, int n_copies, long copy_stride) {
    const long i = (long)blockIdx.x * blockDim.x + threadIdx.x;
    if (i >= (long)B * T * C) return;
    const int c = (int)(i % C);
    const long bt = i / C;
    const int t = (int)(bt % T), b = (int)(bt / T);
    const long o = ((long)b * rows + t) * ldx + c;
    float v = x[o];
    if (t < prompt_len[b]) v = 0.f;
    x[o] = v;
    for (int k = 0; k < n_copies; ++k) x16[k * copy_stride + ((long)b * rows + t) * ldx16 + c] = (half_t)v;
}

__global__ void euler_kernel(float* __restrict__ x, long ldx, half_t* __restrict__ x16, long ldx16, int rows,
                             const float* __restrict__ v, long ldv, long v_stream_stride, int v_off, int B, int T, int C,
                             const int* __restrict__ prompt_len, float dt, float c0, float ca, float cb, int stream_a,
                             int stream_b, int n_copies, long copy_stride) {
    const long i = (long)blockIdx.x * blockDim.x + threadIdx.x;
    if (i >= (long)B * T * C) return;
    const int c = (int)(i % C);
    const long bt = i / C;
    const int t = (int)(bt % T), b = (int)(bt / T);
    const long vo = ((long)b * rows + v_off + t) * ldv + c;
    float d = c0 * v[vo];
    if (stream_a >= 0) d -= ca * v[vo + stream_a * v_stream_stride];
    if (stream_b >= 0) d -= cb * v[vo + stream_b * v_stream_stride];
    const long xo = ((long)b * rows + t) * ldx + c;
    float nx = x[xo] + dt * d;
    if (t < prompt_len[b]) nx = 0.f;
    x[xo] = nx;
    for (int k = 0; k < n_copies; ++k) x16[k * copy_stride + ((long)b * rows + t) * ldx16 + c] = (half_t)nx;
}

__global__ void prompt_rows_kernel(const float* __restrict__ src, int C, int P, float* __restrict__ dst, long ld, int rows,
                                   int T, const int* __restrict__ prompt_len, int B) {
    const long i = (long)blockIdx.x * blockDim.x + threadIdx.x;
    if (i >= (long)B * T * C) return;
    const int t = (int)(i % T);
    const long bc = i / T;
    const int c = (int)(bc % C), b = (int)(bc / C);
    const float v = (t < prompt_len[b] && t < P) ? src[((long)b * C + c) * P + t] : 0.f;
    dst[((long)b * rows + t) * ld + c] = v;
}
}

int svc_dit::run_group(const svc_cfm_args_t* a, int b0, int nb, int n_streams, const int (*flags)[3],
                       const std::vector<float>& tvals, const std::vector<float>& dts, float c0, float ca, float cb,
                       int stream_a, int stream_b, hipStream_t st) {
    const int T = a->T, P = a->P;
    const int n_steps = (int)tvals.size();
    if (reserve(n_streams, nb, T, n_steps, st)) return 1;
    std::vector<int> kv(n_streams * nb), cv(n_streams * nb), pl(nb);
    for (int b = 0; b < nb; ++b) {
        const int len = a->x_lens ? (int)a->x_lens[b0 + b] : T;
        const int plen = a->prompt_lens ? (int)a->prompt_lens[b0 + b] : P;
        SVC_REQUIRE(len >= 1 && len <= T, "x_lens out of range");
        SVC_REQUIRE(plen >= 0 && plen <= P && plen <= len, "prompt_lens out of range");
        pl[b] = plen;
        for (int j = 0; j < n_streams; ++j) {
            kv[j * nb + b] = len + npre;
            cv[j * nb + b] = len;
        }
    }
    {
        int halo = 0;
        if (wavenet) {
            int dil = 1;
            for (int i = 0; i < NL; ++i) {
                const int total = (WK - 1) * dil;
                halo += total - total / 2;
                dil *= cfg.wn_dilation_rate;
            }
        }
        const int min_pl = *std::min_element(pl.begin(), pl.end());
        win0 = std::max(0, npre + min_pl - halo) & ~7;
    }
    std::vector<int> cvw(cv.size());
    for (size_t i = 0; i < cv.size(); ++i) cvw[i] = cv[i] - (win0 - npre > 0 ? win0 - npre : 0);
    {
        const size_t n = kv.size();
        int* h = reinterpret_cast<int*>(staging.acquire((3 * n + pl.size()) * sizeof(int)));
        if (!h) return 1;
        memcpy(h, kv.data(), n * 4); memcpy(h + n, cv.data(), n * 4); memcpy(h + 2 * n, cvw.data(), n * 4);
        memcpy(h + 3 * n, pl.data(), pl.size() * 4);
        SVC_CHECK_HIP(hipMemcpyAsync(d_kvlen, h, n * 4, hipMemcpyHostToDevice, st));
        SVC_CHECK_HIP(hipMemcpyAsync(d_convlen, h + n, n * 4, hipMemcpyHostToDevice, st));
        SVC_CHECK_HIP(hipMemcpyAsync(d_convlen_w, h + 2 * n, n * 4, hipMemcpyHostToDevice, st));
        SVC_CHECK_HIP(hipMemcpyAsync(d_plen, h + 3 * n, pl.size() * 4, hipMemcpyHostToDevice, st));
        if (staging.commit(st)) return 1;
    }
    if (tables(tvals, st)) return 1;

    const long copy_stride = (long)nb * seq_rows * C16;
    const long n_el = (long)nb * T * C;
    if (bct_to_btc_launch(a->z + (long)b0 * C * T, nb, C, T, x32, C16, nullptr, 0, seq_rows, T, a->temperature, st)) return 1;
    hipLaunchKernelGGL(init_state_kernel, dim3(cdiv(n_el, 256)), dim3(256), 0, st, x32, (long)C16, x16, (long)C16, seq_rows,
                       nb, T, C, d_plen, n_streams, copy_stride);
    SVC_CHECK_HIP(hipGetLastError());
    hipLaunchKernelGGL(prompt_rows_kernel, dim3(cdiv(n_el, 256)), dim3(256), 0, st, a->prompt + (long)b0 * C * P, C, P,
                       prompt32, (long)C32, seq_rows, T, d_plen, nb);
    SVC_CHECK_HIP(hipGetLastError());
    if (statics(n_streams, flags, nb, T, a->mu + (long)b0 * T * Dc, a->style + (long)b0 * S, st)) return 1;

    auto steps = [&](hipStream_t s_) -> int {
        for (int s = 0; s < n_steps; ++s) {
            if (body(n_streams, nb, T, s, s_)) return 1;
            hipLaunchKernelGGL(euler_kernel, dim3(cdiv(n_el, 256)), dim3(256), 0, s_, x32, (long)C16, x16, (long)C16, seq_rows,
                               v32, (long)C16, (long)nb * seq_rows * C16, npre, nb, T, C, d_plen, dts[s], c0, ca, cb,
                               stream_a, stream_b, n_streams, copy_stride);
            SVC_CHECK_HIP(hipGetLastError());
        }
        return 0;
    };
    static const int graph_env = [] { const char* e = getenv("SVC_DIT_GRAPH"); return e ? (e[0] == '0' ? 0 : 1) : -1; }();
    bool done = false;
    if ((graph_env >= 0 ? graph_env : use_graphs) && !prof_enabled()) {
        std::vector<float> key = {(float)n_streams, (float)nb, (float)T, (float)n_steps, (float)win0, (float)seq_rows, c0, ca, cb,
                                  (float)stream_a, (float)stream_b, (float)fused_min_rows};
        key.insert(key.end(), dts.begin(), dts.end());
        StepGraph* g = nullptr;
        for (auto& c : graphs) if (c.key == key) { g = &c; break; }
        if (!g) {
            if (graphs.size() >= 8) { if (graphs.front().exec) (void)hipGraphExecDestroy(graphs.front().exec); graphs.erase(graphs.begin()); }
            graphs.push_back(StepGraph());
            g = &graphs.back();
            g->key = key;
        }
        if (g->seen++ >= 1 && !g->exec) {
            if (!cap_stream && hipStreamCreateWithFlags(&cap_stream, hipStreamNonBlocking) != hipSuccess) { (void)hipGetLastError(); cap_stream = nullptr; }
            hipGraph_t gr = nullptr;
            if (cap_stream && hipStreamBeginCapture(cap_stream, hipStreamCaptureModeThreadLocal) == hipSuccess) {
                const int rc = steps(cap_stream);
                const hipError_t e = hipStreamEndCapture(cap_stream, &gr);
                if (rc == 0 && e == hipSuccess && gr && hipGraphInstantiate(&g->exec, gr, nullptr, nullptr, 0) != hipSuccess) g->exec = nullptr;
                if (gr) (void)hipGraphDestroy(gr);
                if (rc || e != hipSuccess) { (void)hipGetLastError(); g->exec = nullptr; if (rc) return 1; }
            } else {
                (void)hipGetLastError();
            }
        }
        if (g->exec) {
            SVC_CHECK_HIP(hipGraphLaunch(g->exec, st));
            done = true;
        }
    }
    if (!done && steps(st)) return 1;
    return btc_to_bct_launch(x32, C16, seq_rows, a->out + (long)b0 * C * T, nb, C, T, st);
}

extern "C" {

int svc_dit_create(const svc_dit_config_t* cfg, const svc_tensor_desc_t* weights, int n_weights, void* stream,
                   svc_dit_t** out) {
    SVC_REQUIRE(cfg && weights && out, "null argument");
    SVC_REQUIRE(cfg->hidden_dim == cfg->num_heads * 64, "head_dim must be 64 (hidden_dim = 64 * num_heads)");
    SVC_REQUIRE(cfg->content_dim % 32 == 0, "content_dim must be a multiple of 32");
    SVC_REQUIRE(cfg->in_channels % 8 == 0 && cfg->in_channels <= 128, "in_channels must be a multiple of 8, <= 128");
    svc_dit* m = new svc_dit();
    m->cfg = *cfg;
    m->device = current_device();
    m->v2 = cfg->version == 2;
    m->D = cfg->hidden_dim; m->H = cfg->num_heads; m->L = cfg->depth; m->C = cfg->in_channels;
    m->Dc = cfg->content_dim; m->S = cfg->style_dim;
    {
        const int n_hidden = (int)(2 * (4 * m->D) / 3);
        m->I = (int)round_up(n_hidden, 256);
    }
    m->wavenet = cfg->final_layer_type == 1;
    m->W = m->wavenet ? cfg->wn_hidden_dim : 0;
    m->NL = m->wavenet ? cfg->wn_num_layers : 0;
    m->WK = m->wavenet ? cfg->wn_kernel_size : 0;
    m->npre = (cfg->time_as_token ? 1 : 0) + (cfg->style_as_token ? 1 : 0);
    m->C16 = (int)round_up(m->C, 64);
    m->C32 = (int)round_up(m->C, 32);
    m->adaptive_blocks = m->v2 || !cfg->time_as_token;
    if (m->wavenet) {
        if (m->W % 64 != 0 || m->W != m->D || m->WK * 1 > KG_MAX_TAPS || m->npre != 0) {
            set_error("wavenet head needs wn_hidden_dim == hidden_dim (FinalLayer modulates with t1), no prefix tokens");
            delete m;
            return 1;
        }
    }
    if (!m->v2 && cfg->uvit_skip_connection) {
        for (int i = 0; i < m->L; ++i) {
            if (i < m->L / 2) m->emit.push_back(i);
            if (i > m->L / 2) m->recv.push_back(i);
        }
    }
    hipStream_t st = (hipStream_t)stream;
    StateDict sd(weights, n_weights);
    if (m->pack(sd, st)) {
        delete m;
        return 1;
    }
    *out = m;
    return 0;
}

void svc_dit_destroy(svc_dit_t* m) {
    if (m) {
        m->drop_graphs();
        if (m->cap_stream) (void)hipStreamDestroy(m->cap_stream);
    }
    delete m;
}

int svc_dit_set_microbatch(svc_dit_t* m, int utterances) {
    SVC_REQUIRE(m && utterances >= 0, "bad argument");
    m->microbatch = utterances;
    return 0;
}

int svc_dit_set_fused_min_rows(svc_dit_t* m, long rows) {
    SVC_REQUIRE(m, "null argument");
    m->fused_min_rows = rows < 0 ? 10240 : rows;
    return 0;
}

int svc_dit_fused_available(svc_dit_t* m) { return m && m->fused_ok ? 1 : 0; }

int svc_dit_set_graphs(svc_dit_t* m, int on) {
    SVC_REQUIRE(m, "null argument");
    m->use_graphs = on ? 1 : 0;
    if (!on) m->drop_graphs();
    return 0;
}

int svc_cfm_sample(svc_dit_t* m, const svc_cfm_args_t* a, void* stream) {
    SVC_REQUIRE(m && a, "null argument");
    SVC_REQUIRE(a->B >= 1 && a->T >= 1 && a->P >= 0 && a->P <= a->T && a->n_timesteps >= 1, "bad sampler shape");
    SVC_REQUIRE(a->T + m->npre <= ROPE_POS, "sequence longer than the RoPE table");
    SVC_REQUIRE(a->mu && (a->prompt || a->P == 0) && a->style && a->z && a->out, "null tensor");
    SVC_REQUIRE(current_device() == m->device, "this handle was created on another device (make it current before the call)");
    hipStream_t st = (hipStream_t)stream;
    const int N = a->n_timesteps;
    std::vector<float> ts = linspace01(N + 1);
    std::vector<float> tvals(N), dts(N);
    if (!m->v2) {
        float t = ts[0];
        for (int s = 1; s <= N; ++s) {
            const float dt = ts[s] - ts[s - 1];
            tvals[s - 1] = t;
            dts[s - 1] = dt;
            t = t + dt;
        }
    } else {
        for (auto& v : ts) v = v + (-1.0f) * (cosf((float)M_PI / 2.0f * v) - 1.0f + v);
        float t = ts[0], dt = ts[1] - ts[0];
        for (int s = 1; s <= N; ++s) {
            tvals[s - 1] = t;
            dts[s - 1] = dt;
            t = t + dt;
            if (s < N) dt = ts[s + 1] - t;
        }
    }
    int flags[MAX_STREAMS][3] = {{1, 1, 1}, {0, 0, 0}, {0, 0, 0}};
    int n_streams = 1, sa = -1, sb = -1;
    float c0 = 1.f, ca = 0.f, cb = 0.f;
    const float ra = a->cfg_rate[0], rb = a->cfg_rate[1];
    if (!m->v2) {
        if (ra > 0.f) { n_streams = 2; sa = 1; c0 = 1.f + ra; ca = ra; }
    } else if (a->random_voice) {
        n_streams = 2; flags[0][0] = 0; flags[0][1] = 0; sa = 1; c0 = 1.f + ra; ca = ra;
    } else if (ra == 0.f && rb == 0.f) {
        n_streams = 1;
    } else if (ra == 0.f) {
        n_streams = 2; flags[1][2] = 1; sa = 1; c0 = 1.f + rb; ca = rb;
    } else if (rb == 0.f) {
        n_streams = 2; sa = 1; c0 = 1.f + ra; ca = ra;
    } else {
        n_streams = 3; flags[1][2] = 1; sa = 2; sb = 1; c0 = 1.f + ra + rb; ca = ra; cb = rb;
    }
    int mb = m->microbatch > 0 ? m->microbatch : 32;
    for (int b0 = 0; b0 < a->B; b0 += mb) {
        const int nb = std::min(mb, a->B - b0);
        if (m->run_group(a, b0, nb, n_streams, flags, tvals, dts, c0, ca, cb, sa, sb, st)) return 1;
    }
    return 0;
}

int svc_dit_forward(svc_dit_t* m, int N, int T, const float* x, const float* prompt_x, const int64_t* x_lens, float t,
                    const float* style, const float* mu, float* out, void* stream) {
    SVC_REQUIRE(m && x && prompt_x && style && mu && out, "null argument");
    SVC_REQUIRE(N >= 1 && T >= 1 && T + m->npre <= ROPE_POS, "bad estimator shape");
    SVC_REQUIRE(current_device() == m->device, "this handle was created on another device (make it current before the call)");
    hipStream_t st = (hipStream_t)stream;
    const int flags[1][3] = {{1, 1, 1}};
    if (m->reserve(1, N, T, 1, st)) return 1;
    std::vector<int> kv(N), cv(N), pl(N);
    for (int b = 0; b < N; ++b) {
        const int len = x_lens ? (int)x_lens[b] : T;
        SVC_REQUIRE(len >= 1 && len <= T, "x_lens out of range");
        kv[b] = len + m->npre; cv[b] = len; pl[b] = T;
    }
    m->win0 = 0;
    {
        int* h = reinterpret_cast<int*>(m->staging.acquire(3 * (size_t)N * sizeof(int)));
        if (!h) return 1;
        memcpy(h, kv.data(), N * 4); memcpy(h + N, cv.data(), N * 4); memcpy(h + 2 * N, pl.data(), N * 4);
        SVC_CHECK_HIP(hipMemcpyAsync(m->d_kvlen, h, N * 4, hipMemcpyHostToDevice, st));
        SVC_CHECK_HIP(hipMemcpyAsync(m->d_convlen, h + N, N * 4, hipMemcpyHostToDevice, st));
        SVC_CHECK_HIP(hipMemcpyAsync(m->d_convlen_w, h + N, N * 4, hipMemcpyHostToDevice, st));
        SVC_CHECK_HIP(hipMemcpyAsync(m->d_plen, h + 2 * N, N * 4, hipMemcpyHostToDevice, st));
        if (m->staging.commit(st)) return 1;
    }
    std::vector<float> tv(1, t);
    if (m->tables(tv, st)) return 1;
    const int C = m->C, C16 = m->C16, C32 = m->C32, rows = m->seq_rows;
    if (bct_to_btc_launch(x, N, C, T, m->x32, C16, m->x16, C16, rows, T, 1.0f, st)) return 1;
    const long n_el = (long)N * T * C;
    hipLaunchKernelGGL(prompt_rows_kernel, dim3(cdiv(n_el, 256)), dim3(256), 0, st, prompt_x, C, T, m->prompt32, (long)C32,
                       rows, T, m->d_plen, N);
    SVC_CHECK_HIP(hipGetLastError());
    if (m->statics(1, flags, N, T, mu, style, st)) return 1;
    if (m->body(1, N, T, 0, st)) return 1;
    return btc_to_bct_launch(m->v32 + (long)m->npre * C16, C16, rows, out, N, C, T, st);
}

}
```

### seed-vc_amd/csrc/fused.hip

```cpp
#include <stdlib.h>

#include <utility>

#include "common.h"

namespace svc {

namespace {

typedef __attribute__((address_space(1))) const void* gptr_t;
typedef __attribute__((address_space(3))) void* lptr_t;

template <int D>
struct PG {
    static constexpr int NT = D / 16;
    static constexpr int KC = D / 32;
    static constexpr int SLOT_BYTES = NT * 1024;
    static constexpr int NS = D == 384 ? 5 : 4;
    static constexpr int RING = NS * SLOT_BYTES;
    static constexpr int PF = D == 384 ? 6 : 4;
    static constexpr int NVEC = 9;
    static constexpr int LDS = RING + NVEC * D * 4;
};

__device__ __forceinline__ half8 frag_read(unsigned lds_addr, int off) {
    half8 r;
    asm volatile("ds_read_b128 %0, %1 offset:%2" : "=v"(r) : "v"(lds_addr), "n"(0) : "memory");
    (void)off;
    return r;
}
template <int OFF>
__device__ __forceinline__ void frag_read_to(half8& r, unsigned lds_addr) {
    asm volatile("ds_read_b128 %0, %1 offset:%2" : "=v"(r) : "v"(lds_addr), "n"(OFF));
}
template <int N>
__device__ __forceinline__ void frag_wait(half8& r) {
    asm volatile("s_waitcnt lgkmcnt(%1)" : "+v"(r) : "n"(N));
}

template <int NF, int PF, int TM, int RFI, typename F, typename R>
__device__ __forceinline__ void stream_frags(const char* base, F&& body, R&& refill) {
    static_assert(NF * 1024 <= 65536 && PF >= 1 && PF <= 8, "ds_read offset field");
    const unsigned la = (unsigned)(uintptr_t)(lptr_t)const_cast<char*>(base);
    half8 q[PF];
    [&]<int... I>(std::integer_sequence<int, I...>) { (frag_read_to<I * 1024>(q[I], la), ...); }(std::make_integer_sequence<int, PF>{});
    [&]<int... Fi>(std::integer_sequence<int, Fi...>) {
        ([&] {
            constexpr int f = Fi;
            constexpr int pending = (NF - f < PF ? NF - f : PF) - 1;
            frag_wait<pending>(q[f % PF]);
            const half8 w = q[f % PF];
            body(f, w);
            if constexpr (f + PF < NF) frag_read_to<(f + PF) * 1024>(q[f % PF], la);
            if constexpr (f % RFI == RFI - 1) refill(f / RFI);
            __builtin_amdgcn_sched_barrier(0);
        }(), ...);
    }(std::make_integer_sequence<int, NF>{});
}

__device__ __forceinline__ void mfma_v(float4v& c, const half8 a, const half8 b) {
    asm volatile("v_mfma_f32_16x16x32_f16 %0, %1, %2, %0" : "+v"(c) : "v"(a), "v"(b));
}
__device__ __forceinline__ void mfma_guard(float4v (&a)[4][2]) {
    asm volatile("s_nop 15\n\ts_nop 3"
                 : "+v"(a[0][0]), "+v"(a[0][1]), "+v"(a[1][0]), "+v"(a[1][1]), "+v"(a[2][0]), "+v"(a[2][1]), "+v"(a[3][0]), "+v"(a[3][1]));
}
__device__ __forceinline__ void mfma_guard(float4v (&a)[4][1]) {}
template <int NF, typename F, typename R>
__device__ __forceinline__ void stream_frags_asm(const char* base, F&& body, R&& refill) {
    static_assert(NF % 4 == 0, "fragment groups of 4");
    half8 q[2][4];
#pragma unroll
    for (int i = 0; i < 4; ++i) q[0][i] = *reinterpret_cast<const half8*>(base + i * 1024);
#pragma unroll
    for (int g = 0; g < NF / 4; ++g) {
        if (g + 1 < NF / 4) {
#pragma unroll
            for (int i = 0; i < 4; ++i) q[(g + 1) & 1][i] = *reinterpret_cast<const half8*>(base + ((g + 1) * 4 + i) * 1024);
        }
        __builtin_amdgcn_sched_barrier(0);
#pragma unroll
        for (int i = 0; i < 4; ++i) body(g * 4 + i, q[g & 1][i]);
        refill(g);
        __builtin_amdgcn_sched_barrier(0);
    }
}

enum { V_AF = 0, V_BF = 1, V_GA = 2, V_GF = 3, V_AA = 4, V_BA = 5, V_BS = 6, V_AN = 7, V_BN = 8 };

template <int D, bool GATED, int TM>
__global__ __launch_bounds__(128 / (16 * TM) * 64, 128 / (16 * TM) / 4) void dit_panel_kernel(const PanelParams p) {
    using G = PG<D>;
    constexpr int NT = G::NT, KC = G::KC, NS = G::NS, PF = G::PF;
    constexpr int NW = 128 / (16 * TM), NTHR = NW * 64, DPS = NT / NW, RFI = NT / DPS;
    constexpr bool ASM_SIDE = D == 512 && TM == 2;
    extern __shared__ __attribute__((aligned(16))) char smem[];
    float* vec = reinterpret_cast<float*>(smem + G::RING);

    const int tid = threadIdx.x, lane = tid & 63;
    const int wave = __builtin_amdgcn_readfirstlane(tid >> 6);
    const int fr = lane & 15, fq = lane >> 4;
    const int m0 = blockIdx.x * 128 + wave * (16 * TM);

    for (int c = tid; c < D; c += NTHR) {
        const float one = p.add_one ? 1.f : 0.f;
        vec[V_AF * D + c] = p.g_ffn ? p.g_ffn[c] * (p.w_f ? one + p.w_f[c] : 1.f) : 0.f;
        vec[V_BF * D + c] = p.b_f ? p.b_f[c] : 0.f;
        vec[V_GA * D + c] = p.gate_a ? p.gate_a[c] : 1.f;
        vec[V_GF * D + c] = p.gate_f ? p.gate_f[c] : 1.f;
        vec[V_AA * D + c] = p.g_attn ? p.g_attn[c] * (p.w_a ? one + p.w_a[c] : 1.f) : 0.f;
        vec[V_BA * D + c] = p.b_a ? p.b_a[c] : 0.f;
        vec[V_BS * D + c] = p.bskip ? p.bskip[c] : 0.f;
        vec[V_AN * D + c] = p.g_fin ? p.g_fin[c] * (p.w_fin ? one + p.w_fin[c] : 1.f) : 0.f;
        vec[V_BN * D + c] = p.b_fin ? p.b_fin[c] : 0.f;
    }
    __syncthreads();

    const char* wsrc = reinterpret_cast<const char*>(p.wstream) + wave * (G::SLOT_BYTES / NW) + lane * 16;
    int s_next = 0, stage = 0, fill = NS - 1, s_issued = 0;
    auto piece = [&](const char* src, char* dst, int i) {
        const char* s4 = src + (i >> 2) * 4096;
        char* d4 = dst + (i >> 2) * 4096;
        switch (i & 3) {
            case 0: __builtin_amdgcn_global_load_lds((gptr_t)s4, (lptr_t)d4, 16, 0, 0); break;
            case 1: __builtin_amdgcn_global_load_lds((gptr_t)s4, (lptr_t)d4, 16, 1024, 0); break;
            case 2: __builtin_amdgcn_global_load_lds((gptr_t)s4, (lptr_t)d4, 16, 2048, 0); break;
            default: __builtin_amdgcn_global_load_lds((gptr_t)s4, (lptr_t)d4, 16, 3072, 0); break;
        }
    };
    const char* rf_src = nullptr;
    char* rf_dst = nullptr;
    auto acquire = [&]() -> const char* {
        const int ahead = p.n_slots - 1 - s_next;
        if constexpr (NS == 5) {
            if (ahead >= 3) asm volatile("s_waitcnt vmcnt(%0)" ::"n"(3 * DPS) : "memory");
            else if (ahead == 2) asm volatile("s_waitcnt vmcnt(%0)" ::"n"(2 * DPS) : "memory");
            else if (ahead == 1) asm volatile("s_waitcnt vmcnt(%0)" ::"n"(DPS) : "memory");
            else asm volatile("s_waitcnt vmcnt(0)" ::: "memory");
        } else {
            if (ahead >= 2) asm volatile("s_waitcnt vmcnt(%0)" ::"n"(2 * DPS) : "memory");
            else if (ahead == 1) asm volatile("s_waitcnt vmcnt(%0)" ::"n"(DPS) : "memory");
            else asm volatile("s_waitcnt vmcnt(0)" ::: "memory");
        }
        asm volatile("s_barrier" ::: "memory");
        const int src_slot = s_issued < p.n_slots ? s_issued : p.n_slots - 1;
        rf_src = wsrc + (long)src_slot * G::SLOT_BYTES;
        rf_dst = smem + fill * G::SLOT_BYTES + wave * (G::SLOT_BYTES / NW);
        ++s_issued;
        const char* ptr = smem + stage * G::SLOT_BYTES + lane * 16;
        stage = stage + 1 == NS ? 0 : stage + 1;
        fill = fill + 1 == NS ? 0 : fill + 1;
        ++s_next;
        return ptr;
    };
    auto refill = [&](int i) { piece(rf_src, rf_dst, i); };
#define FRAG(base, idx) (*reinterpret_cast<const half8*>((base) + (idx) * 1024))
#define MFMA(a, b, c) __builtin_amdgcn_mfma_f32_16x16x32_f16((a), (b), (c), 0, 0, 0)

#pragma unroll
    for (int s_ = 0; s_ < NS - 1; ++s_) {
        const int src_slot = s_ < p.n_slots ? s_ : p.n_slots - 1;
#pragma unroll
        for (int i = 0; i < DPS; ++i)
            piece(wsrc + (long)src_slot * G::SLOT_BYTES, smem + s_ * G::SLOT_BYTES + wave * (G::SLOT_BYTES / NW), i);
        ++s_issued;
    }

    long grow[TM];
    bool rok[TM];
#pragma unroll
    for (int mt = 0; mt < TM; ++mt) {
        const int m = m0 + 16 * mt + fr;
        rok[mt] = m < p.M;
        const int mm = rok[mt] ? m : p.M - 1;
        const int seq = mm / p.Lout;
        grow[mt] = (long)seq * p.seq_rows + p.row_off + (mm - seq * p.Lout);
    }

    float4v acc[NT][TM];
    half8 xn[KC][TM];

    auto norm_to_xn = [&](const float* va, const float* vb) {
        float rs[TM];
#pragma unroll
        for (int mt = 0; mt < TM; ++mt) {
            float ss = 0.f;
#pragma unroll
            for (int t = 0; t < NT; ++t)
#pragma unroll
                for (int r = 0; r < 4; ++r) ss += acc[t][mt][r] * acc[t][mt][r];
            ss += __shfl_xor(ss, 16);
            ss += __shfl_xor(ss, 32);
            rs[mt] = rsqrtf(ss / (float)D + p.eps);
        }
#pragma unroll
        for (int c = 0; c < KC; ++c) {
            const float4v a0 = *reinterpret_cast<const float4v*>(va + 32 * c + 4 * fq);
            const float4v a1 = *reinterpret_cast<const float4v*>(va + 32 * c + 16 + 4 * fq);
            const float4v b0 = *reinterpret_cast<const float4v*>(vb + 32 * c + 4 * fq);
            const float4v b1 = *reinterpret_cast<const float4v*>(vb + 32 * c + 16 + 4 * fq);
#pragma unroll
            for (int mt = 0; mt < TM; ++mt) {
                half8 h;
#pragma unroll
                for (int j = 0; j < 4; ++j) {
                    h[j] = (half_t)(acc[2 * c][mt][j] * rs[mt] * a0[j] + b0[j]);
                    h[4 + j] = (half_t)(acc[2 * c + 1][mt][j] * rs[mt] * a1[j] + b1[j]);
                }
                xn[c][mt] = h;
            }
        }
    };
    auto store_x = [&]() {
#pragma unroll
        for (int mt = 0; mt < TM; ++mt)
            if (rok[mt]) {
#pragma unroll
                for (int t = 0; t < NT; ++t) *reinterpret_cast<float4v*>(p.x + grow[mt] * D + 16 * t + 4 * fq) = acc[t][mt];
            }
    };

    if (p.do_post) {
        {
            half8 af[KC][TM];
#pragma unroll
            for (int mt = 0; mt < TM; ++mt) {
#pragma unroll
                for (int kc = 0; kc < KC; ++kc)
                    af[kc][mt] = *reinterpret_cast<const half8*>(p.ao + grow[mt] * D + 32 * kc + 8 * fq);
#pragma unroll
                for (int t = 0; t < NT; ++t)
                    acc[t][mt] = GATED ? (float4v){0.f, 0.f, 0.f, 0.f}
                                       : *reinterpret_cast<const float4v*>(p.x + grow[mt] * D + 16 * t + 4 * fq);
            }
#pragma unroll
            for (int kc = 0; kc < KC; ++kc) {
                const char* base = acquire();
                stream_frags<NT, PF, TM, RFI>(base, [&](int t, half8 w) {
#pragma unroll
                    for (int mt = 0; mt < TM; ++mt) acc[t][mt] = MFMA(w, af[kc][mt], acc[t][mt]);
                }, refill);
            }
        }
        if constexpr (GATED) {
#pragma unroll
            for (int mt = 0; mt < TM; ++mt)
#pragma unroll
                for (int t = 0; t < NT; ++t) {
                    const float4v xi = *reinterpret_cast<const float4v*>(p.x + grow[mt] * D + 16 * t + 4 * fq);
                    const float4v ga = *reinterpret_cast<const float4v*>(vec + V_GA * D + 16 * t + 4 * fq);
#pragma unroll
                    for (int r = 0; r < 4; ++r) acc[t][mt][r] = xi[r] + ga[r] * acc[t][mt][r];
                }
            store_x();
        }
        norm_to_xn(vec + V_AF * D, vec + V_BF * D);
        if constexpr (GATED) {
#pragma unroll
            for (int mt = 0; mt < TM; ++mt)
#pragma unroll
                for (int t = 0; t < NT; ++t) acc[t][mt] = (float4v){0.f, 0.f, 0.f, 0.f};
        }
        const int n_chunks = p.I / 32;
        for (int c = 0; c < n_chunks; ++c) {
            float4v a1[4][TM];
#pragma unroll
            for (int t = 0; t < 4; ++t)
#pragma unroll
                for (int mt = 0; mt < TM; ++mt) a1[t][mt] = (float4v){0.f, 0.f, 0.f, 0.f};
            {
                const char* base = acquire();
                if constexpr (ASM_SIDE) {
                    stream_frags_asm<NT>(base, [&](int f, half8 w) {
                        _Pragma("unroll") for (int mt = 0; mt < TM; ++mt) mfma_v(a1[f & 3][mt], w, xn[f >> 2][mt]);
                    }, refill);
                } else {
                    stream_frags<NT, PF, TM, RFI>(base, [&](int f, half8 w) {
                        _Pragma("unroll") for (int mt = 0; mt < TM; ++mt) a1[f & 3][mt] = MFMA(w, xn[f >> 2][mt], a1[f & 3][mt]);
                    }, refill);
                }
            }
            {
                const char* base = acquire();
                if constexpr (ASM_SIDE) {
                    stream_frags_asm<NT>(base, [&](int f, half8 w) {
                        _Pragma("unroll") for (int mt = 0; mt < TM; ++mt) mfma_v(a1[f & 3][mt], w, xn[KC / 2 + (f >> 2)][mt]);
                    }, refill);
                    mfma_guard(a1);
                } else {
                    stream_frags<NT, PF, TM, RFI>(base, [&](int f, half8 w) {
                        _Pragma("unroll") for (int mt = 0; mt < TM; ++mt) a1[f & 3][mt] = MFMA(w, xn[KC / 2 + (f >> 2)][mt], a1[f & 3][mt]);
                    }, refill);
                }
            }
            half8 hf[TM];
            constexpr float LOG2E = 1.4426950408889634f;
#pragma unroll
            for (int mt = 0; mt < TM; ++mt)
#pragma unroll
                for (int t = 0; t < 4; ++t)
#pragma unroll
                    for (int i = 0; i < 2; ++i) {
                        const float a = a1[t][mt][2 * i], b = a1[t][mt][2 * i + 1];
                        hf[mt][2 * t + i] = (half_t)(a * __builtin_amdgcn_rcpf(1.0f + __builtin_amdgcn_exp2f(-a * LOG2E)) * b);
                    }
            {
                const char* base = acquire();
                stream_frags<NT, PF, TM, RFI>(base, [&](int t, half8 w) {
#pragma unroll
                    for (int mt = 0; mt < TM; ++mt) acc[t][mt] = MFMA(w, hf[mt], acc[t][mt]);
                }, refill);
            }
        }
        if constexpr (GATED) {
#pragma unroll
            for (int mt = 0; mt < TM; ++mt)
#pragma unroll
                for (int t = 0; t < NT; ++t) {
                    const float4v xi = *reinterpret_cast<const float4v*>(p.x + grow[mt] * D + 16 * t + 4 * fq);
                    const float4v gf = *reinterpret_cast<const float4v*>(vec + V_GF * D + 16 * t + 4 * fq);
#pragma unroll
                    for (int r = 0; r < 4; ++r) acc[t][mt][r] = xi[r] + gf[r] * acc[t][mt][r];
                }
        }
        if (!p.do_skip) store_x();
        if (p.c16) {
#pragma unroll
            for (int mt = 0; mt < TM; ++mt)
                if (rok[mt]) {
#pragma unroll
                    for (int t = 0; t < NT; ++t) {
                        const half4 h = {(half_t)acc[t][mt][0], (half_t)acc[t][mt][1], (half_t)acc[t][mt][2], (half_t)acc[t][mt][3]};
                        *reinterpret_cast<half4*>(p.c16 + grow[mt] * D + 16 * t + 4 * fq) = h;
                    }
                }
        }
    } else {
#pragma unroll
        for (int mt = 0; mt < TM; ++mt)
#pragma unroll
            for (int t = 0; t < NT; ++t) acc[t][mt] = *reinterpret_cast<const float4v*>(p.x + grow[mt] * D + 16 * t + 4 * fq);
    }

    if (p.do_skip) {
#pragma unroll
        for (int c = 0; c < KC; ++c)
#pragma unroll
            for (int mt = 0; mt < TM; ++mt) {
                half8 h;
#pragma unroll
                for (int j = 0; j < 4; ++j) {
                    h[j] = (half_t)acc[2 * c][mt][j];
                    h[4 + j] = (half_t)acc[2 * c + 1][mt][j];
                }
                xn[c][mt] = h;
            }
#pragma unroll
        for (int t = 0; t < NT; ++t)
#pragma unroll
            for (int mt = 0; mt < TM; ++mt) acc[t][mt] = *reinterpret_cast<const float4v*>(vec + V_BS * D + 16 * t + 4 * fq);
#pragma unroll
        for (int kc = 0; kc < KC; ++kc) {
            const char* base = acquire();
            stream_frags<NT, PF, TM, RFI>(base, [&](int t, half8 w) {
#pragma unroll
                for (int mt = 0; mt < TM; ++mt) acc[t][mt] = MFMA(w, xn[kc][mt], acc[t][mt]);
            }, refill);
        }
#pragma unroll
        for (int mt = 0; mt < TM; ++mt)
#pragma unroll
            for (int kc = 0; kc < KC; ++kc)
                xn[kc][mt] = *reinterpret_cast<const half8*>(p.skip_in + grow[mt] * D + 32 * kc + 8 * fq);
#pragma unroll
        for (int kc = 0; kc < KC; ++kc) {
            const char* base = acquire();
            stream_frags<NT, PF, TM, RFI>(base, [&](int t, half8 w) {
#pragma unroll
                for (int mt = 0; mt < TM; ++mt) acc[t][mt] = MFMA(w, xn[kc][mt], acc[t][mt]);
            }, refill);
        }
        store_x();
    }

    if (p.do_final) {
        float rs[TM];
#pragma unroll
        for (int mt = 0; mt < TM; ++mt) {
            float ss = 0.f;
#pragma unroll
            for (int t = 0; t < NT; ++t)
#pragma unroll
                for (int r = 0; r < 4; ++r) ss += acc[t][mt][r] * acc[t][mt][r];
            ss += __shfl_xor(ss, 16);
            ss += __shfl_xor(ss, 32);
            rs[mt] = rsqrtf(ss / (float)D + p.eps);
        }
#pragma unroll
        for (int t = 0; t < NT; ++t) {
            const float4v a = *reinterpret_cast<const float4v*>(vec + V_AN * D + 16 * t + 4 * fq);
            const float4v b = *reinterpret_cast<const float4v*>(vec + V_BN * D + 16 * t + 4 * fq);
#pragma unroll
            for (int mt = 0; mt < TM; ++mt)
                if (rok[mt]) {
                    half4 h;
#pragma unroll
                    for (int r = 0; r < 4; ++r) h[r] = (half_t)(acc[t][mt][r] * rs[mt] * a[r] + b[r]);
                    *reinterpret_cast<half4*>(p.n16 + grow[mt] * D + 16 * t + 4 * fq) = h;
                }
        }
    }

    if (p.do_qkv) {
        norm_to_xn(vec + V_AA * D, vec + V_BA * D);
        float rp[TM][16];
        int posl[TM];
#pragma unroll
        for (int mt = 0; mt < TM; ++mt) {
            const int m = m0 + 16 * mt + fr;
            const int mm = m < p.M ? m : p.M - 1;
            posl[mt] = p.row_off + mm % p.Lout;
            const float* tb = p.rope + ((long)posl[mt] * 32 + 8 * fq) * 2;
#pragma unroll
            for (int q4 = 0; q4 < 4; ++q4) {
                const float4v t4 = *reinterpret_cast<const float4v*>(tb + 4 * q4);
#pragma unroll
                for (int j = 0; j < 4; ++j) rp[mt][4 * q4 + j] = t4[j];
            }
        }
        const int n_groups = 3 * D / 64, n_qk = 2 * D / 64;
        for (int grp = 0; grp < n_groups; ++grp) {
            float4v a1[4][TM];
#pragma unroll
            for (int t = 0; t < 4; ++t)
#pragma unroll
                for (int mt = 0; mt < TM; ++mt) a1[t][mt] = (float4v){0.f, 0.f, 0.f, 0.f};
            if (grp < n_qk) {
#pragma unroll
                for (int hs = 0; hs < 2; ++hs) {
                    const char* base = acquire();
                    if constexpr (ASM_SIDE) {
                        stream_frags_asm<NT>(base, [&](int f, half8 w) {
                            _Pragma("unroll") for (int mt = 0; mt < TM; ++mt) mfma_v(a1[f & 3][mt], w, xn[hs * (KC / 2) + (f >> 2)][mt]);
                        }, refill);
                        if (hs == 1) mfma_guard(a1);
                    } else {
                        stream_frags<NT, PF, TM, RFI>(base, [&](int f, half8 w) {
                            _Pragma("unroll") for (int mt = 0; mt < TM; ++mt) a1[f & 3][mt] = MFMA(w, xn[hs * (KC / 2) + (f >> 2)][mt], a1[f & 3][mt]);
                        }, refill);
                    }
                }
                const float sc = grp < D / 64 ? p.q_scale : 1.0f;
#pragma unroll
                for (int mt = 0; mt < TM; ++mt) {
                    float o[16];
#pragma unroll
                    for (int i = 0; i < 8; ++i) {
                        const float x0 = a1[i >> 1][mt][2 * (i & 1)], x1 = a1[i >> 1][mt][2 * (i & 1) + 1];
                        const float cs = rp[mt][2 * i], sn = rp[mt][2 * i + 1];
                        o[2 * i] = (x0 * cs - x1 * sn) * sc;
                        o[2 * i + 1] = (x1 * cs + x0 * sn) * sc;
                    }
                    if (rok[mt]) {
                        half_t* dst = p.qk + grow[mt] * (2 * D) + 64 * grp + 16 * fq;
                        *reinterpret_cast<uint4*>(dst) = pack8(o);
                        *reinterpret_cast<uint4*>(dst + 8) = pack8(o + 8);
                    }
                }
            } else {
#pragma unroll
                for (int hs = 0; hs < 2; ++hs) {
                    const char* base = acquire();
                    if constexpr (ASM_SIDE) {
                        stream_frags_asm<NT>(base, [&](int f, half8 w) {
                            _Pragma("unroll") for (int mt = 0; mt < TM; ++mt) mfma_v(a1[f & 3][mt], xn[hs * (KC / 2) + (f >> 2)][mt], w);
                        }, refill);
                        if (hs == 1) mfma_guard(a1);
                    } else {
                        stream_frags<NT, PF, TM, RFI>(base, [&](int f, half8 w) {
                            _Pragma("unroll") for (int mt = 0; mt < TM; ++mt) a1[f & 3][mt] = MFMA(xn[hs * (KC / 2) + (f >> 2)][mt], w, a1[f & 3][mt]);
                        }, refill);
                    }
                }
#pragma unroll
                for (int mt = 0; mt < TM; ++mt) {
                    const int m = m0 + 16 * mt + 4 * fq;
                    if (m < p.M) {
                        const int seq = m / p.Lout;
                        const int pos = p.row_off + (m - seq * p.Lout);
#pragma unroll
                        for (int t = 0; t < 4; ++t) {
                            const int d = 64 * (grp - n_qk) + 16 * t + fr;
                            const half4 h = {(half_t)a1[t][mt][0], (half_t)a1[t][mt][1], (half_t)a1[t][mt][2], (half_t)a1[t][mt][3]};
                            *reinterpret_cast<half4*>(p.vt + (long)seq * p.vt_seq_stride + (long)d * p.vt_ld + vt_pos(pos, p.vt_mode ? p.vt_mode : 1)) = h;
                        }
                    }
                }
            }
        }
    }
    asm volatile("s_waitcnt vmcnt(0)" ::: "memory");
#undef FRAG
#undef MFMA
}

__global__ void pack_stream_kernel(half_t* __restrict__ dst, long n_elems, int mode, int D, int I, const float* __restrict__ w0,
                                   const float* __restrict__ w1, const float* __restrict__ w2) {
    const long e = (long)blockIdx.x * blockDim.x + threadIdx.x;
    if (e >= n_elems) return;
    const int NT = D / 16, KC = D / 32;
    const long f = e >> 9;
    const int l = (int)((e >> 3) & 63), j = (int)(e & 7);
    const int fr = l & 15, g = l >> 4;
    const int kperm = 16 * (j >> 2) + 4 * g + (j & 3);
    const int knat = 8 * g + j;
    float v = 0.f;
    if (mode == 0) {
        const int kc = (int)(f / NT), t = (int)(f % NT);
        v = w0[(long)(16 * t + fr) * D + 32 * kc + knat];
    } else if (mode == 1) {
        const long per = 3L * NT;
        const int c = (int)(f / per), q = (int)(f % per);
        if (q < 2 * NT) {
            const int kc = q / 4, t = q % 4;
            const int h = 32 * c + 8 * (fr >> 2) + 2 * t + ((fr & 3) >> 1);
            const float* src = (fr & 1) ? w1 : w0;
            v = src[(long)h * D + 32 * kc + kperm];
        } else {
            const int t = q - 2 * NT;
            v = w2[(long)(16 * t + fr) * I + 32 * c + knat];
        }
    } else if (mode == 2) {
        const int kc = (int)(f / NT), t = (int)(f % NT);
        const int k = kc < KC ? 32 * kc + kperm : D + 32 * (kc - KC) + knat;
        v = w0[(long)(16 * t + fr) * (2 * D) + k];
    } else {
        const int grp = (int)(f / (4 * KC)), q = (int)(f % (4 * KC));
        const int kc = q / 4, t = q % 4;
        const int n = grp < 2 * D / 64 ? 64 * grp + 16 * (fr >> 2) + 4 * t + (fr & 3) : 64 * grp + 16 * t + fr;
        v = w0[(long)n * D + 32 * kc + kperm];
    }
    dst[e] = (half_t)v;
}

}

bool fused_supported(int D, int I) {
    static const bool off = [] { const char* e = getenv("SVC_FUSED"); return e && e[0] == '0'; }();
    return !off && (D == 384 || D == 512) && I % 32 == 0;
}

static long slots_post(int D, int I) { return D / 32 + 3L * (I / 32); }
static long slots_skip(int D) { return 2L * (D / 32); }
static long slots_qkv(int D) { return 2L * (3 * D / 64); }

long fused_stream_halfs(int D, int I, bool post, bool skip, bool qkv) {
    const long slot_halfs = (long)(D / 16) * 512;
    return ((post ? slots_post(D, I) : 0) + (skip ? slots_skip(D) : 0) + (qkv ? slots_qkv(D) : 0)) * slot_halfs;
}

long fused_pack_stream(half_t* dst, int D, int I, const float* wo, const float* w1, const float* w3, const float* w2,
                       const float* wskip, const float* wqkv, hipStream_t st) {
    const long slot_halfs = (long)(D / 16) * 512;
    long off = 0;
    auto run = [&](int mode, long slots, const float* a, const float* b, const float* c) -> bool {
        const long n = slots * slot_halfs;
        hipLaunchKernelGGL(pack_stream_kernel, dim3(cdiv(n, 256)), dim3(256), 0, st, dst + off, n, mode, D, I, a, b, c);
        off += n;
        return hipGetLastError() == hipSuccess;
    };
    if (wo) {
        if (!run(0, D / 32, wo, nullptr, nullptr)) return 0;
        if (!run(1, 3L * (I / 32), w1, w3, w2)) return 0;
    }
    if (wskip && !run(2, slots_skip(D), wskip, nullptr, nullptr)) return 0;
    if (wqkv && !run(3, slots_qkv(D), wqkv, nullptr, nullptr)) return 0;
    return off;
}

int fused_panel_launch(const PanelParams& p, int D, bool gated, hipStream_t st) {
    SVC_REQUIRE(D == 384 || D == 512, "fused panel kernel: D must be 384 or 512");
    SVC_REQUIRE(p.M > 0 && p.Lout > 0 && p.I % 32 == 0, "fused panel kernel: shape");
    SVC_REQUIRE(!p.do_qkv || (p.M % 4 == 0 && p.Lout % 4 == 0 && p.row_off % 4 == 0), "fused panel kernel: v^T stores need 4-row groups");
    DeviceState* ds = device_state();
    if (!ds) return 1;
    if (!ds->fused_attr.load(std::memory_order_acquire)) {
#define SVC_PANEL_ATTR(DD, GG, TT) SVC_CHECK_HIP(hipFuncSetAttribute(reinterpret_cast<const void*>(dit_panel_kernel<DD, GG, TT>), hipFuncAttributeMaxDynamicSharedMemorySize, PG<DD>::LDS))
        SVC_PANEL_ATTR(384, false, 1); SVC_PANEL_ATTR(384, true, 1); SVC_PANEL_ATTR(512, false, 1); SVC_PANEL_ATTR(512, true, 1);
        SVC_PANEL_ATTR(384, false, 2); SVC_PANEL_ATTR(384, true, 2); SVC_PANEL_ATTR(512, false, 2); SVC_PANEL_ATTR(512, true, 2);
#undef SVC_PANEL_ATTR
        ds->fused_attr.store(true, std::memory_order_release);
    }
    const long want = (p.do_post ? slots_post(D, p.I) : 0) + (p.do_skip ? slots_skip(D) : 0) + (p.do_qkv ? slots_qkv(D) : 0);
    SVC_REQUIRE(want == p.n_slots, "fused panel kernel: slot count does not match the enabled phases");
    const int grid = cdiv(p.M, 128);
    const bool prof = prof_enabled();
    if (prof) prof_begin(PROF_FUSED, st);
    static const int tm_env = [] { const char* e = getenv("SVC_FUSED_TM"); return e ? atoi(e) : 0; }();
    const int tm = (tm_env == 1 || tm_env == 2) ? tm_env : (D == 384 ? 2 : 1);
#define SVC_PANEL_LAUNCH(DD, GG, TT) hipLaunchKernelGGL((dit_panel_kernel<DD, GG, TT>), dim3(grid), dim3(128 / (16 * TT) * 64), PG<DD>::LDS, st, p)
    if (tm == 2) {
        if (D == 384) { if (gated) SVC_PANEL_LAUNCH(384, true, 2); else SVC_PANEL_LAUNCH(384, false, 2); }
        else { if (gated) SVC_PANEL_LAUNCH(512, true, 2); else SVC_PANEL_LAUNCH(512, false, 2); }
    } else {
        if (D == 384) { if (gated) SVC_PANEL_LAUNCH(384, true, 1); else SVC_PANEL_LAUNCH(384, false, 1); }
        else { if (gated) SVC_PANEL_LAUNCH(512, true, 1); else SVC_PANEL_LAUNCH(512, false, 1); }
    }
#undef SVC_PANEL_LAUNCH
    SVC_CHECK_HIP(hipGetLastError());
    if (prof) {
        const double M = p.M, Dd = D;
        double macs = 0;
        if (p.do_post) macs += Dd * Dd + 3.0 * Dd * p.I;
        if (p.do_skip) macs += 2.0 * Dd * Dd;
        if (p.do_qkv) macs += 3.0 * Dd * Dd;
        double bytes = 2.0 * macs;
        bytes += M * Dd * ((p.do_post ? 4 + 2 : 4) + ((p.do_post && !p.do_skip) || p.do_skip ? 4 : 0) + (p.c16 ? 2 : 0) +
                           (p.do_skip ? 2 : 0) + (p.do_qkv ? 6 : 0) + (p.do_final ? 2 : 0));
        const unsigned long long tag = ((unsigned long long)p.M << 40) | ((unsigned long long)(D & 0xFFFFF) << 20) |
                                       ((unsigned long long)(p.I & 0xFFFF) << 4) |
                                       (unsigned)((p.do_post ? 1 : 0) | (p.do_skip ? 2 : 0) | (p.do_qkv ? 4 : 0) | (p.do_final ? 8 : 0));
        prof_end(PROF_FUSED, 2.0 * M * macs, bytes, st, tag);
    }
    return 0;
}

}
```

Baseline: 138,100 mel-frames/s.

## Make fused DiT panel kernel persistent with cross-panel weight ring and residual prefetch

Turns the fused panel kernel into a persistent kernel. The grid is capped at the CU count by default and each block loops over several 128-row panels. The weight-stream ring keeps refilling from the start of the stream for the next panel, so the pipeline does not drain between panels. For the non-gated D=384 variant, the next panel's residual rows are prefetched into the accumulators during the QKV phase, with adjusted vmcnt waits. The aim is to remove per-block launch and pipeline fill/drain costs and hide the latency of the residual load, at the cost of more complex wait accounting and a new grid knob added to the graph cache key.

After: 137,700 mel-frames/s, median of 2. Within noise of the previous version (-0.3%).

```diff
diff --git a/include/seedvc_hip.h b/include/seedvc_hip.h
--- a/include/seedvc_hip.h
+++ b/include/seedvc_hip.h
@@ -33,6 +33,7 @@
 int svc_dit_set_microbatch(svc_dit_t* m, int utterances);
 
 int svc_dit_set_fused_min_rows(svc_dit_t* m, long rows);
+int svc_dit_set_panel_grid(svc_dit_t* m, int n);
 int svc_dit_fused_available(svc_dit_t* m);
 int svc_dit_set_graphs(svc_dit_t* m, int on);
 
diff --git a/seed-vc_amd/_lib.py b/seed-vc_amd/_lib.py
--- a/seed-vc_amd/_lib.py
+++ b/seed-vc_amd/_lib.py
@@ -8,7 +8,7 @@
 
 EXPORTS = [
     "svc_abi_version", "svc_last_error",
-    "svc_dit_create", "svc_dit_destroy", "svc_dit_set_microbatch", "svc_dit_set_fused_min_rows", "svc_dit_fused_available", "svc_dit_set_graphs", "svc_cfm_sample", "svc_dit_forward",
+    "svc_dit_create", "svc_dit_destroy", "svc_dit_set_microbatch", "svc_dit_set_fused_min_rows", "svc_dit_set_panel_grid", "svc_dit_fused_available", "svc_dit_set_graphs", "svc_cfm_sample", "svc_dit_forward",
     "svc_bigvgan_create", "svc_bigvgan_destroy", "svc_bigvgan_forward", "svc_bigvgan_forward_ragged", "svc_bigvgan_set_microbatch",
     "svc_hift_create", "svc_hift_destroy", "svc_hift_forward", "svc_hift_forward_ragged", "svc_hift_set_microbatch",
     "svc_anti_alias_act_fwd",
diff --git a/seed-vc_amd/cfm.py b/seed-vc_amd/cfm.py
--- a/seed-vc_amd/cfm.py
+++ b/seed-vc_amd/cfm.py
@@ -44,6 +44,9 @@
 
     def set_fused_min_rows(self, rows):
         _lib.check(_lib.lib().svc_dit_set_fused_min_rows(self._h, C.c_long(int(rows))))
+
+    def set_panel_grid(self, n):
+        _lib.check(_lib.lib().svc_dit_set_panel_grid(self._h, int(n)))
 
     def set_graphs(self, on):
         _lib.check(_lib.lib().svc_dit_set_graphs(self._h, int(bool(on))))
diff --git a/seed-vc_amd/csrc/common.h b/seed-vc_amd/csrc/common.h
--- a/seed-vc_amd/csrc/common.h
+++ b/seed-vc_amd/csrc/common.h
@@ -53,6 +53,7 @@
     void* zero_page = nullptr;
     std::atomic<unsigned long long> kconv_attr{0};
     std::atomic<bool> fused_attr{false};
+    int n_cus = 0;
 };
 DeviceState* device_state();
 int current_device();
@@ -203,7 +204,7 @@
 long fused_stream_halfs(int D, int I, bool post, bool skip, bool qkv);
 long fused_pack_stream(half_t* dst, int D, int I, const float* wo, const float* w1, const float* w3, const float* w2,
                        const float* wskip, const float* wqkv, hipStream_t st);
-int fused_panel_launch(const PanelParams& p, int D, bool gated, hipStream_t st);
+int fused_panel_launch(const PanelParams& p, int D, bool gated, hipStream_t st, int panel_grid = 0);
 
 struct AttnParams {
     const half_t* q; const half_t* k; long ld_qk;
diff --git a/seed-vc_amd/csrc/device.hip b/seed-vc_amd/csrc/device.hip
--- a/seed-vc_amd/csrc/device.hip
+++ b/seed-vc_amd/csrc/device.hip
@@ -27,8 +27,15 @@
         set_error("device_state: zero page allocation failed");
         return nullptr;
     }
+    hipDeviceProp_t prop;
+    if (hipGetDeviceProperties(&prop, d) != hipSuccess) {
+        (void)hipFree(zp);
+        set_error("device_state: hipGetDeviceProperties failed");
+        return nullptr;
+    }
     DeviceState* s = new DeviceState();
     s->device = d;
+    s->n_cus = prop.multiProcessorCount;
     s->zero_page = zp;
     states[d] = s;
     return s;
diff --git a/seed-vc_amd/csrc/dit.hip b/seed-vc_amd/csrc/dit.hip
--- a/seed-vc_amd/csrc/dit.hip
+++ b/seed-vc_amd/csrc/dit.hip
@@ -59,6 +59,7 @@
     half_t* stream_pre = nullptr;
     int stream_pre_slots = 0;
     bool fused_ok = false;
+    int panel_grid = 0;
     long fused_min_rows = 10240;
     std::vector<Layer> layers;
     float* g_final;
@@ -823,7 +824,7 @@
         PanelParams p = base();
         p.wstream = stream_pre; p.n_slots = stream_pre_slots;
         set_qkv(p, 0);
-        if (fused_panel_launch(p, D, v2, st)) return 1;
+        if (fused_panel_launch(p, D, v2, st, panel_grid)) return 1;
     }
     size_t emit_i = 0;
     std::vector<int> skip_stack;
@@ -865,7 +866,7 @@
             p.do_final = 1; p.g_fin = g_final; p.w_fin = fm; p.b_fin = fm + D; p.n16 = n16;
             if (tail_only) { p.Lout = seq_rows - win0; p.row_off = win0; p.M = nseq * p.Lout; }
         }
-        if (fused_panel_launch(p, D, v2, st)) return 1;
+        if (fused_panel_launch(p, D, v2, st, panel_grid)) return 1;
     }
     return 0;
 }
@@ -1031,7 +1032,7 @@
     bool done = false;
     if ((graph_env >= 0 ? graph_env : use_graphs) && !prof_enabled()) {
         std::vector<float> key = {(float)n_streams, (float)nb, (float)T, (float)n_steps, (float)win0, (float)seq_rows, c0, ca, cb,
-                                  (float)stream_a, (float)stream_b, (float)fused_min_rows};
+                                  (float)stream_a, (float)stream_b, (float)fused_min_rows, (float)panel_grid};
         key.insert(key.end(), dts.begin(), dts.end());
         StepGraph* g = nullptr;
         for (auto& c : graphs) if (c.key == key) { g = &c; break; }
@@ -1129,6 +1130,12 @@
 int svc_dit_set_fused_min_rows(svc_dit_t* m, long rows) {
     SVC_REQUIRE(m, "null argument");
     m->fused_min_rows = rows < 0 ? 10240 : rows;
+    return 0;
+}
+
+int svc_dit_set_panel_grid(svc_dit_t* m, int n) {
+    SVC_REQUIRE(m && n >= -1, "bad argument");
+    m->panel_grid = n;
     return 0;
 }
 
diff --git a/seed-vc_amd/csrc/fused.hip b/seed-vc_amd/csrc/fused.hip
--- a/seed-vc_amd/csrc/fused.hip
+++ b/seed-vc_amd/csrc/fused.hip
@@ -86,21 +86,29 @@
     }
 }
 
+template <int D, int TM> struct PrefetchBursts { static constexpr int b[5] = {0, 0, 0, 0, 0}; };
+template <> struct PrefetchBursts<384, 2> { static constexpr int b[5] = {0, 0, 8, 28, 48}; };
+template <> struct PrefetchBursts<384, 1> { static constexpr int b[5] = {0, 0, 4, 14, 24}; };
+
 enum { V_AF = 0, V_BF = 1, V_GA = 2, V_GF = 3, V_AA = 4, V_BA = 5, V_BS = 6, V_AN = 7, V_BN = 8 };
 
 template <int D, bool GATED, int TM>
-__global__ __launch_bounds__(128 / (16 * TM) * 64, 128 / (16 * TM) / 4) void dit_panel_kernel(const PanelParams p) {
+__global__ __launch_bounds__(128 / (16 * TM) * 64, 128 / (16 * TM) / 4) void dit_panel_kernel(const PanelParams p0) {
     using G = PG<D>;
     constexpr int NT = G::NT, KC = G::KC, NS = G::NS, PF = G::PF;
     constexpr int NW = 128 / (16 * TM), NTHR = NW * 64, DPS = NT / NW, RFI = NT / DPS;
     constexpr bool ASM_SIDE = D == 512 && TM == 2;
+    constexpr bool PREFETCH = !GATED && D == 384;
+    constexpr const int* PFB = PrefetchBursts<D, TM>::b;
     extern __shared__ __attribute__((aligned(16))) char smem[];
     float* vec = reinterpret_cast<float*>(smem + G::RING);
 
-    const int tid = threadIdx.x, lane = tid & 63;
+    const int tid = threadIdx.x, lane0 = tid & 63;
     const int wave = __builtin_amdgcn_readfirstlane(tid >> 6);
-    const int fr = lane & 15, fq = lane >> 4;
-    const int m0 = blockIdx.x * 128 + wave * (16 * TM);
+    typedef const __attribute__((address_space(4))) PanelParams kparams_t;
+    kparams_t* pk = (kparams_t*)__builtin_amdgcn_kernarg_segment_ptr();
+    const PanelParams& p = p0;
+    const int n_panels = (p.M + 127) >> 7;
 
     for (int c = tid; c < D; c += NTHR) {
         const float one = p.add_one ? 1.f : 0.f;
@@ -116,8 +124,11 @@
     }
     __syncthreads();
 
-    const char* wsrc = reinterpret_cast<const char*>(p.wstream) + wave * (G::SLOT_BYTES / NW) + lane * 16;
+    const char* wsrc = reinterpret_cast<const char*>(p.wstream) + wave * (G::SLOT_BYTES / NW) + lane0 * 16;
     int s_next = 0, stage = 0, fill = NS - 1, s_issued = 0;
+    bool has_next = false;
+    int burst = 0;
+    int boost = 0;
     auto piece = [&](const char* src, char* dst, int i) {
         const char* s4 = src + (i >> 2) * 4096;
         char* d4 = dst + (i >> 2) * 4096;
@@ -131,8 +142,14 @@
     const char* rf_src = nullptr;
     char* rf_dst = nullptr;
     auto acquire = [&]() -> const char* {
-        const int ahead = p.n_slots - 1 - s_next;
-        if constexpr (NS == 5) {
+        const int ahead = has_next ? NS : p.n_slots - 1 - s_next;
+        if (boost > 0) {
+            if (burst == 0) asm volatile("s_waitcnt vmcnt(%0)" ::"n"((NS - 2) * DPS + PFB[1] - PFB[0]) : "memory");
+            else if (burst == 1) asm volatile("s_waitcnt vmcnt(%0)" ::"n"((NS - 2) * DPS + PFB[2] - PFB[1]) : "memory");
+            else if (burst == 2) asm volatile("s_waitcnt vmcnt(%0)" ::"n"((NS - 2) * DPS + PFB[3] - PFB[2]) : "memory");
+            else asm volatile("s_waitcnt vmcnt(%0)" ::"n"((NS - 2) * DPS + PFB[4] - PFB[3]) : "memory");
+            --boost;
+        } else if constexpr (NS == 5) {
             if (ahead >= 3) asm volatile("s_waitcnt vmcnt(%0)" ::"n"(3 * DPS) : "memory");
             else if (ahead == 2) asm volatile("s_waitcnt vmcnt(%0)" ::"n"(2 * DPS) : "memory");
             else if (ahead == 1) asm volatile("s_waitcnt vmcnt(%0)" ::"n"(DPS) : "memory");
@@ -143,11 +160,11 @@
             else asm volatile("s_waitcnt vmcnt(0)" ::: "memory");
         }
         asm volatile("s_barrier" ::: "memory");
-        const int src_slot = s_issued < p.n_slots ? s_issued : p.n_slots - 1;
+        const int src_slot = s_issued < p.n_slots ? s_issued : (has_next ? s_issued - p.n_slots : p.n_slots - 1);
         rf_src = wsrc + (long)src_slot * G::SLOT_BYTES;
         rf_dst = smem + fill * G::SLOT_BYTES + wave * (G::SLOT_BYTES / NW);
         ++s_issued;
-        const char* ptr = smem + stage * G::SLOT_BYTES + lane * 16;
+        const char* ptr = smem + stage * G::SLOT_BYTES + lane0 * 16;
         stage = stage + 1 == NS ? 0 : stage + 1;
         fill = fill + 1 == NS ? 0 : fill + 1;
         ++s_next;
@@ -163,279 +180,299 @@
 #pragma unroll
         for (int i = 0; i < DPS; ++i)
             piece(wsrc + (long)src_slot * G::SLOT_BYTES, smem + s_ * G::SLOT_BYTES + wave * (G::SLOT_BYTES / NW), i);
-        ++s_issued;
-    }
-
-    long grow[TM];
-    bool rok[TM];
-#pragma unroll
-    for (int mt = 0; mt < TM; ++mt) {
-        const int m = m0 + 16 * mt + fr;
-        rok[mt] = m < p.M;
-        const int mm = rok[mt] ? m : p.M - 1;
-        const int seq = mm / p.Lout;
-        grow[mt] = (long)seq * p.seq_rows + p.row_off + (mm - seq * p.Lout);
     }
 
     float4v acc[NT][TM];
-    half8 xn[KC][TM];
-
-    auto norm_to_xn = [&](const float* va, const float* vb) {
-        float rs[TM];
+    bool have_x = false;
+
+    for (int panel = blockIdx.x; panel < n_panels; panel += gridDim.x) {
+        int lane = lane0;
+        asm volatile("" : "+v"(lane));
+        kparams_t& p = *pk;
+        const int fr = lane & 15, fq = lane >> 4;
+        const int m0 = panel * 128 + wave * (16 * TM);
+        has_next = panel + (int)gridDim.x < n_panels;
+        s_next = 0;
+        s_issued = NS - 1;
+        bool pref = false;
+        long grow[TM];
+        bool rok[TM];
 #pragma unroll
         for (int mt = 0; mt < TM; ++mt) {
-            float ss = 0.f;
+            const int m = m0 + 16 * mt + fr;
+            rok[mt] = m < p.M;
+            const int mm = rok[mt] ? m : p.M - 1;
+            const int seq = mm / p.Lout;
+            grow[mt] = (long)seq * p.seq_rows + p.row_off + (mm - seq * p.Lout);
+        }
+
+        half8 xn[KC][TM];
+
+        auto norm_to_xn = [&](const float* va, const float* vb) {
+            float rs[TM];
+#pragma unroll
+            for (int mt = 0; mt < TM; ++mt) {
+                float ss = 0.f;
+#pragma unroll
+                for (int t = 0; t < NT; ++t)
+#pragma unroll
+                    for (int r = 0; r < 4; ++r) ss += acc[t][mt][r] * acc[t][mt][r];
+                ss += __shfl_xor(ss, 16);
+                ss += __shfl_xor(ss, 32);
+                rs[mt] = rsqrtf(ss / (float)D + p.eps);
+            }
+#pragma unroll
+            for (int c = 0; c < KC; ++c) {
+                const float4v a0 = *reinterpret_cast<const float4v*>(va + 32 * c + 4 * fq);
+                const float4v a1 = *reinterpret_cast<const float4v*>(va + 32 * c + 16 + 4 * fq);
+                const float4v b0 = *reinterpret_cast<const float4v*>(vb + 32 * c + 4 * fq);
+                const float4v b1 = *reinterpret_cast<const float4v*>(vb + 32 * c + 16 + 4 * fq);
+#pragma unroll
+                for (int mt = 0; mt < TM; ++mt) {
+                    half8 h;
+#pragma unroll
+                    for (int j = 0; j < 4; ++j) {
+                        h[j] = (half_t)(acc[2 * c][mt][j] * rs[mt] * a0[j] + b0[j]);
+                        h[4 + j] = (half_t)(acc[2 * c + 1][mt][j] * rs[mt] * a1[j] + b1[j]);
+                    }
+                    xn[c][mt] = h;
+                }
+            }
+        };
+        auto store_x = [&]() {
+#pragma unroll
+            for (int mt = 0; mt < TM; ++mt)
+                if (rok[mt]) {
+#pragma unroll
+                    for (int t = 0; t < NT; ++t) *reinterpret_cast<float4v*>(p.x + grow[mt] * D + 16 * t + 4 * fq) = acc[t][mt];
+                }
+        };
+
+        if (p.do_post) {
+            {
+                half8 af[KC][TM];
+#pragma unroll
+                for (int mt = 0; mt < TM; ++mt) {
+#pragma unroll
+                    for (int kc = 0; kc < KC; ++kc)
+                        af[kc][mt] = *reinterpret_cast<const half8*>(p.ao + grow[mt] * D + 32 * kc + 8 * fq);
+                    if constexpr (!PREFETCH) {
+#pragma unroll
+                        for (int t = 0; t < NT; ++t)
+                            acc[t][mt] = GATED ? (float4v){0.f, 0.f, 0.f, 0.f}
+                                               : *reinterpret_cast<const float4v*>(p.x + grow[mt] * D + 16 * t + 4 * fq);
+                    }
+                }
+                if constexpr (PREFETCH) {
+                    if (!have_x) {
+#pragma unroll
+                        for (int mt = 0; mt < TM; ++mt)
+#pragma unroll
+                            for (int t = 0; t < NT; ++t) acc[t][mt] = *reinterpret_cast<const float4v*>(p.x + grow[mt] * D + 16 * t + 4 * fq);
+                    }
+                }
+#pragma unroll
+                for (int kc = 0; kc < KC; ++kc) {
+                    const char* base = acquire();
+                    stream_frags<NT, PF, TM, RFI>(base, [&](int t, half8 w) {
+#pragma unroll
+                        for (int mt = 0; mt < TM; ++mt) acc[t][mt] = MFMA(w, af[kc][mt], acc[t][mt]);
+                    }, refill);
+                }
+            }
+            if constexpr (GATED) {
+#pragma unroll
+                for (int mt = 0; mt < TM; ++mt)
+#pragma unroll
+                    for (int t = 0; t < NT; ++t) {
+                        const float4v xi = *reinterpret_cast<const float4v*>(p.x + grow[mt] * D + 16 * t + 4 * fq);
+                        const float4v ga = *reinterpret_cast<const float4v*>(vec + V_GA * D + 16 * t + 4 * fq);
+#pragma unroll
+                        for (int r = 0; r < 4; ++r) acc[t][mt][r] = xi[r] + ga[r] * acc[t][mt][r];
+                    }
+                store_x();
+            }
+            norm_to_xn(vec + V_AF * D, vec + V_BF * D);
+            if constexpr (GATED) {
+#pragma unroll
+                for (int mt = 0; mt < TM; ++mt)
+#pragma unroll
+                    for (int t = 0; t < NT; ++t) acc[t][mt] = (float4v){0.f, 0.f, 0.f, 0.f};
+            }
+            const int n_chunks = p.I / 32;
+            for (int c = 0; c < n_chunks; ++c) {
+                float4v a1[4][TM];
+#pragma unroll
+                for (int t = 0; t < 4; ++t)
+#pragma unroll
+                    for (int mt = 0; mt < TM; ++mt) a1[t][mt] = (float4v){0.f, 0.f, 0.f, 0.f};
+                {
+                    const char* base = acquire();
+                    if constexpr (ASM_SIDE) {
+                        stream_frags_asm<NT>(base, [&](int f, half8 w) {
+                            _Pragma("unroll") for (int mt = 0; mt < TM; ++mt) mfma_v(a1[f & 3][mt], w, xn[f >> 2][mt]);
+                        }, refill);
+                    } else {
+                        stream_frags<NT, PF, TM, RFI>(base, [&](int f, half8 w) {
+                            _Pragma("unroll") for (int mt = 0; mt < TM; ++mt) a1[f & 3][mt] = MFMA(w, xn[f >> 2][mt], a1[f & 3][mt]);
+                        }, refill);
+                    }
+                }
+                {
+                    const char* base = acquire();
+                    if constexpr (ASM_SIDE) {
+                        stream_frags_asm<NT>(base, [&](int f, half8 w) {
+                            _Pragma("unroll") for (int mt = 0; mt < TM; ++mt) mfma_v(a1[f & 3][mt], w, xn[KC / 2 + (f >> 2)][mt]);
+                        }, refill);
+                        mfma_guard(a1);
+                    } else {
+                        stream_frags<NT, PF, TM, RFI>(base, [&](int f, half8 w) {
+                            _Pragma("unroll") for (int mt = 0; mt < TM; ++mt) a1[f & 3][mt] = MFMA(w, xn[KC / 2 + (f >> 2)][mt], a1[f & 3][mt]);
+                        }, refill);
+                    }
+                }
+                half8 hf[TM];
+                constexpr float LOG2E = 1.4426950408889634f;
+#pragma unroll
+                for (int mt = 0; mt < TM; ++mt)
+#pragma unroll
+                    for (int t = 0; t < 4; ++t)
+#pragma unroll
+                        for (int i = 0; i < 2; ++i) {
+                            const float a = a1[t][mt][2 * i], b = a1[t][mt][2 * i + 1];
+                            hf[mt][2 * t + i] = (half_t)(a * __builtin_amdgcn_rcpf(1.0f + __builtin_amdgcn_exp2f(-a * LOG2E)) * b);
+                        }
+                {
+                    const char* base = acquire();
+                    stream_frags<NT, PF, TM, RFI>(base, [&](int t, half8 w) {
+#pragma unroll
+                        for (int mt = 0; mt < TM; ++mt) acc[t][mt] = MFMA(w, hf[mt], acc[t][mt]);
+                    }, refill);
+                }
+            }
+            if constexpr (GATED) {
+#pragma unroll
+                for (int mt = 0; mt < TM; ++mt)
+#pragma unroll
+                    for (int t = 0; t < NT; ++t) {
+                        const float4v xi = *reinterpret_cast<const float4v*>(p.x + grow[mt] * D + 16 * t + 4 * fq);
+                        const float4v gf = *reinterpret_cast<const float4v*>(vec + V_GF * D + 16 * t + 4 * fq);
+#pragma unroll
+                        for (int r = 0; r < 4; ++r) acc[t][mt][r] = xi[r] + gf[r] * acc[t][mt][r];
+                    }
+            }
+            if (!p.do_skip) store_x();
+            if (p.c16) {
+#pragma unroll
+                for (int mt = 0; mt < TM; ++mt)
+                    if (rok[mt]) {
+#pragma unroll
+                        for (int t = 0; t < NT; ++t) {
+                            const half4 h = {(half_t)acc[t][mt][0], (half_t)acc[t][mt][1], (half_t)acc[t][mt][2], (half_t)acc[t][mt][3]};
+                            *reinterpret_cast<half4*>(p.c16 + grow[mt] * D + 16 * t + 4 * fq) = h;
+                        }
+                    }
+            }
+        } else {
+#pragma unroll
+            for (int mt = 0; mt < TM; ++mt)
+#pragma unroll
+                for (int t = 0; t < NT; ++t) acc[t][mt] = *reinterpret_cast<const float4v*>(p.x + grow[mt] * D + 16 * t + 4 * fq);
+        }
+
+        if (p.do_skip) {
+#pragma unroll
+            for (int c = 0; c < KC; ++c)
+#pragma unroll
+                for (int mt = 0; mt < TM; ++mt) {
+                    half8 h;
+#pragma unroll
+                    for (int j = 0; j < 4; ++j) {
+                        h[j] = (half_t)acc[2 * c][mt][j];
+                        h[4 + j] = (half_t)acc[2 * c + 1][mt][j];
+                    }
+                    xn[c][mt] = h;
+                }
 #pragma unroll
             for (int t = 0; t < NT; ++t)
 #pragma unroll
-                for (int r = 0; r < 4; ++r) ss += acc[t][mt][r] * acc[t][mt][r];
-            ss += __shfl_xor(ss, 16);
-            ss += __shfl_xor(ss, 32);
-            rs[mt] = rsqrtf(ss / (float)D + p.eps);
-        }
-#pragma unroll
-        for (int c = 0; c < KC; ++c) {
-            const float4v a0 = *reinterpret_cast<const float4v*>(va + 32 * c + 4 * fq);
-            const float4v a1 = *reinterpret_cast<const float4v*>(va + 32 * c + 16 + 4 * fq);
-            const float4v b0 = *reinterpret_cast<const float4v*>(vb + 32 * c + 4 * fq);
-            const float4v b1 = *reinterpret_cast<const float4v*>(vb + 32 * c + 16 + 4 * fq);
-#pragma unroll
-            for (int mt = 0; mt < TM; ++mt) {
-                half8 h;
-#pragma unroll
-                for (int j = 0; j < 4; ++j) {
-                    h[j] = (half_t)(acc[2 * c][mt][j] * rs[mt] * a0[j] + b0[j]);
-                    h[4 + j] = (half_t)(acc[2 * c + 1][mt][j] * rs[mt] * a1[j] + b1[j]);
-                }
-                xn[c][mt] = h;
-            }
-        }
-    };
-    auto store_x = [&]() {
-#pragma unroll
-        for (int mt = 0; mt < TM; ++mt)
-            if (rok[mt]) {
-#pragma unroll
-                for (int t = 0; t < NT; ++t) *reinterpret_cast<float4v*>(p.x + grow[mt] * D + 16 * t + 4 * fq) = acc[t][mt];
-            }
-    };
-
-    if (p.do_post) {
-        {
-            half8 af[KC][TM];
-#pragma unroll
-            for (int mt = 0; mt < TM; ++mt) {
-#pragma unroll
-                for (int kc = 0; kc < KC; ++kc)
-                    af[kc][mt] = *reinterpret_cast<const half8*>(p.ao + grow[mt] * D + 32 * kc + 8 * fq);
-#pragma unroll
-                for (int t = 0; t < NT; ++t)
-                    acc[t][mt] = GATED ? (float4v){0.f, 0.f, 0.f, 0.f}
-                                       : *reinterpret_cast<const float4v*>(p.x + grow[mt] * D + 16 * t + 4 * fq);
-            }
+                for (int mt = 0; mt < TM; ++mt) acc[t][mt] = *reinterpret_cast<const float4v*>(vec + V_BS * D + 16 * t + 4 * fq);
 #pragma unroll
             for (int kc = 0; kc < KC; ++kc) {
                 const char* base = acquire();
                 stream_frags<NT, PF, TM, RFI>(base, [&](int t, half8 w) {
 #pragma unroll
-                    for (int mt = 0; mt < TM; ++mt) acc[t][mt] = MFMA(w, af[kc][mt], acc[t][mt]);
+                    for (int mt = 0; mt < TM; ++mt) acc[t][mt] = MFMA(w, xn[kc][mt], acc[t][mt]);
                 }, refill);
             }
-        }
-        if constexpr (GATED) {
 #pragma unroll
             for (int mt = 0; mt < TM; ++mt)
 #pragma unroll
-                for (int t = 0; t < NT; ++t) {
-                    const float4v xi = *reinterpret_cast<const float4v*>(p.x + grow[mt] * D + 16 * t + 4 * fq);
-                    const float4v ga = *reinterpret_cast<const float4v*>(vec + V_GA * D + 16 * t + 4 * fq);
-#pragma unroll
-                    for (int r = 0; r < 4; ++r) acc[t][mt][r] = xi[r] + ga[r] * acc[t][mt][r];
-                }
-            store_x();
-        }
-        norm_to_xn(vec + V_AF * D, vec + V_BF * D);
-        if constexpr (GATED) {
-#pragma unroll
-            for (int mt = 0; mt < TM; ++mt)
-#pragma unroll
-                for (int t = 0; t < NT; ++t) acc[t][mt] = (float4v){0.f, 0.f, 0.f, 0.f};
-        }
-        const int n_chunks = p.I / 32;
-        for (int c = 0; c < n_chunks; ++c) {
-            float4v a1[4][TM];
-#pragma unroll
-            for (int t = 0; t < 4; ++t)
-#pragma unroll
-                for (int mt = 0; mt < TM; ++mt) a1[t][mt] = (float4v){0.f, 0.f, 0.f, 0.f};
-            {
-                const char* base = acquire();
-                if constexpr (ASM_SIDE) {
-                    stream_frags_asm<NT>(base, [&](int f, half8 w) {
-                        _Pragma("unroll") for (int mt = 0; mt < TM; ++mt) mfma_v(a1[f & 3][mt], w, xn[f >> 2][mt]);
-                    }, refill);
-                } else {
-                    stream_frags<NT, PF, TM, RFI>(base, [&](int f, half8 w) {
-                        _Pragma("unroll") for (int mt = 0; mt < TM; ++mt) a1[f & 3][mt] = MFMA(w, xn[f >> 2][mt], a1[f & 3][mt]);
-                    }, refill);
-                }
-            }
-            {
-                const char* base = acquire();
-                if constexpr (ASM_SIDE) {
-                    stream_frags_asm<NT>(base, [&](int f, half8 w) {
-                        _Pragma("unroll") for (int mt = 0; mt < TM; ++mt) mfma_v(a1[f & 3][mt], w, xn[KC / 2 + (f >> 2)][mt]);
-                    }, refill);
-                    mfma_guard(a1);
-                } else {
-                    stream_frags<NT, PF, TM, RFI>(base, [&](int f, half8 w) {
-                        _Pragma("unroll") for (int mt = 0; mt < TM; ++mt) a1[f & 3][mt] = MFMA(w, xn[KC / 2 + (f >> 2)][mt], a1[f & 3][mt]);
-                    }, refill);
-                }
-            }
-            half8 hf[TM];
-            constexpr float LOG2E = 1.4426950408889634f;
-#pragma unroll
-            for (int mt = 0; mt < TM; ++mt)
-#pragma unroll
-                for (int t = 0; t < 4; ++t)
-#pragma unroll
-                    for (int i = 0; i < 2; ++i) {
-                        const float a = a1[t][mt][2 * i], b = a1[t][mt][2 * i + 1];
-                        hf[mt][2 * t + i] = (half_t)(a * __builtin_amdgcn_rcpf(1.0f + __builtin_amdgcn_exp2f(-a * LOG2E)) * b);
-                    }
-            {
+                for (int kc = 0; kc < KC; ++kc)
+                    xn[kc][mt] = *reinterpret_cast<const half8*>(p.skip_in + grow[mt] * D + 32 * kc + 8 * fq);
+#pragma unroll
+            for (int kc = 0; kc < KC; ++kc) {
                 const char* base = acquire();
                 stream_frags<NT, PF, TM, RFI>(base, [&](int t, half8 w) {
 #pragma unroll
-                    for (int mt = 0; mt < TM; ++mt) acc[t][mt] = MFMA(w, hf[mt], acc[t][mt]);
+                    for (int mt = 0; mt < TM; ++mt) acc[t][mt] = MFMA(w, xn[kc][mt], acc[t][mt]);
                 }, refill);
             }
-        }
-        if constexpr (GATED) {
-#pragma unroll
-            for (int mt = 0; mt < TM; ++mt)
-#pragma unroll
-                for (int t = 0; t < NT; ++t) {
-                    const float4v xi = *reinterpret_cast<const float4v*>(p.x + grow[mt] * D + 16 * t + 4 * fq);
-                    const float4v gf = *reinterpret_cast<const float4v*>(vec + V_GF * D + 16 * t + 4 * fq);
-#pragma unroll
-                    for (int r = 0; r < 4; ++r) acc[t][mt][r] = xi[r] + gf[r] * acc[t][mt][r];
-                }
-        }
-        if (!p.do_skip) store_x();
-        if (p.c16) {
-#pragma unroll
-            for (int mt = 0; mt < TM; ++mt)
-                if (rok[mt]) {
-#pragma unroll
-                    for (int t = 0; t < NT; ++t) {
-                        const half4 h = {(half_t)acc[t][mt][0], (half_t)acc[t][mt][1], (half_t)acc[t][mt][2], (half_t)acc[t][mt][3]};
-                        *reinterpret_cast<half4*>(p.c16 + grow[mt] * D + 16 * t + 4 * fq) = h;
-                    }
-                }
-        }
-    } else {
-#pragma unroll
-        for (int mt = 0; mt < TM; ++mt)
-#pragma unroll
-            for (int t = 0; t < NT; ++t) acc[t][mt] = *reinterpret_cast<const float4v*>(p.x + grow[mt] * D + 16 * t + 4 * fq);
-    }
-
-    if (p.do_skip) {
-#pragma unroll
-        for (int c = 0; c < KC; ++c)
+            store_x();
+        }
+
+        if (p.do_final) {
+            float rs[TM];
 #pragma unroll
             for (int mt = 0; mt < TM; ++mt) {
-                half8 h;
-#pragma unroll
-                for (int j = 0; j < 4; ++j) {
-                    h[j] = (half_t)acc[2 * c][mt][j];
-                    h[4 + j] = (half_t)acc[2 * c + 1][mt][j];
-                }
-                xn[c][mt] = h;
-            }
-#pragma unroll
-        for (int t = 0; t < NT; ++t)
-#pragma unroll
-            for (int mt = 0; mt < TM; ++mt) acc[t][mt] = *reinterpret_cast<const float4v*>(vec + V_BS * D + 16 * t + 4 * fq);
-#pragma unroll
-        for (int kc = 0; kc < KC; ++kc) {
-            const char* base = acquire();
-            stream_frags<NT, PF, TM, RFI>(base, [&](int t, half8 w) {
-#pragma unroll
-                for (int mt = 0; mt < TM; ++mt) acc[t][mt] = MFMA(w, xn[kc][mt], acc[t][mt]);
-            }, refill);
-        }
-#pragma unroll
-        for (int mt = 0; mt < TM; ++mt)
-#pragma unroll
-            for (int kc = 0; kc < KC; ++kc)
-                xn[kc][mt] = *reinterpret_cast<const half8*>(p.skip_in + grow[mt] * D + 32 * kc + 8 * fq);
-#pragma unroll
-        for (int kc = 0; kc < KC; ++kc) {
-            const char* base = acquire();
-            stream_frags<NT, PF, TM, RFI>(base, [&](int t, half8 w) {
-#pragma unroll
-                for (int mt = 0; mt < TM; ++mt) acc[t][mt] = MFMA(w, xn[kc][mt], acc[t][mt]);
-            }, refill);
-        }
-        store_x();
-    }
-
-    if (p.do_final) {
-        float rs[TM];
-#pragma unroll
-        for (int mt = 0; mt < TM; ++mt) {
-            float ss = 0.f;
-#pragma unroll
-            for (int t = 0; t < NT; ++t)
-#pragma unroll
-                for (int r = 0; r < 4; ++r) ss += acc[t][mt][r] * acc[t][mt][r];
-            ss += __shfl_xor(ss, 16);
-            ss += __shfl_xor(ss, 32);
-            rs[mt] = rsqrtf(ss / (float)D + p.eps);
-        }
-#pragma unroll
-        for (int t = 0; t < NT; ++t) {
-            const float4v a = *reinterpret_cast<const float4v*>(vec + V_AN * D + 16 * t + 4 * fq);
-            const float4v b = *reinterpret_cast<const float4v*>(vec + V_BN * D + 16 * t + 4 * fq);
-#pragma unroll
-            for (int mt = 0; mt < TM; ++mt)
-                if (rok[mt]) {
-                    half4 h;
-#pragma unroll
-                    for (int r = 0; r < 4; ++r) h[r] = (half_t)(acc[t][mt][r] * rs[mt] * a[r] + b[r]);
-                    *reinterpret_cast<half4*>(p.n16 + grow[mt] * D + 16 * t + 4 * fq) = h;
-                }
-        }
-    }
-
-    if (p.do_qkv) {
-        norm_to_xn(vec + V_AA * D, vec + V_BA * D);
-        float rp[TM][16];
-        int posl[TM];
-#pragma unroll
-        for (int mt = 0; mt < TM; ++mt) {
-            const int m = m0 + 16 * mt + fr;
-            const int mm = m < p.M ? m : p.M - 1;
-            posl[mt] = p.row_off + mm % p.Lout;
-            const float* tb = p.rope + ((long)posl[mt] * 32 + 8 * fq) * 2;
-#pragma unroll
-            for (int q4 = 0; q4 < 4; ++q4) {
-                const float4v t4 = *reinterpret_cast<const float4v*>(tb + 4 * q4);
-#pragma unroll
-                for (int j = 0; j < 4; ++j) rp[mt][4 * q4 + j] = t4[j];
-            }
-        }
-        const int n_groups = 3 * D / 64, n_qk = 2 * D / 64;
-        for (int grp = 0; grp < n_groups; ++grp) {
-            float4v a1[4][TM];
-#pragma unroll
-            for (int t = 0; t < 4; ++t)
-#pragma unroll
-                for (int mt = 0; mt < TM; ++mt) a1[t][mt] = (float4v){0.f, 0.f, 0.f, 0.f};
-            if (grp < n_qk) {
+                float ss = 0.f;
+#pragma unroll
+                for (int t = 0; t < NT; ++t)
+#pragma unroll
+                    for (int r = 0; r < 4; ++r) ss += acc[t][mt][r] * acc[t][mt][r];
+                ss += __shfl_xor(ss, 16);
+                ss += __shfl_xor(ss, 32);
+                rs[mt] = rsqrtf(ss / (float)D + p.eps);
+            }
+#pragma unroll
+            for (int t = 0; t < NT; ++t) {
+                const float4v a = *reinterpret_cast<const float4v*>(vec + V_AN * D + 16 * t + 4 * fq);
+                const float4v b = *reinterpret_cast<const float4v*>(vec + V_BN * D + 16 * t + 4 * fq);
+#pragma unroll
+                for (int mt = 0; mt < TM; ++mt)
+                    if (rok[mt]) {
+                        half4 h;
+#pragma unroll
+                        for (int r = 0; r < 4; ++r) h[r] = (half_t)(acc[t][mt][r] * rs[mt] * a[r] + b[r]);
+                        *reinterpret_cast<half4*>(p.n16 + grow[mt] * D + 16 * t + 4 * fq) = h;
+                    }
+            }
+        }
+
+        if (p.do_qkv) {
+            norm_to_xn(vec + V_AA * D, vec + V_BA * D);
+            float rp[TM][16];
+            int posl[TM];
+#pragma unroll
+            for (int mt = 0; mt < TM; ++mt) {
+                const int m = m0 + 16 * mt + fr;
+                const int mm = m < p.M ? m : p.M - 1;
+                posl[mt] = p.row_off + mm % p.Lout;
+                const float* tb = p.rope + ((long)posl[mt] * 32 + 8 * fq) * 2;
+#pragma unroll
+                for (int q4 = 0; q4 < 4; ++q4) {
+                    const float4v t4 = *reinterpret_cast<const float4v*>(tb + 4 * q4);
+#pragma unroll
+                    for (int j = 0; j < 4; ++j) rp[mt][4 * q4 + j] = t4[j];
+                }
+            }
+            constexpr int n_groups = 3 * D / 64, n_qk = 2 * D / 64;
+            auto qk_group = [&](int grp) {
+                float4v a1[4][TM];
+#pragma unroll
+                for (int t = 0; t < 4; ++t)
+#pragma unroll
+                    for (int mt = 0; mt < TM; ++mt) a1[t][mt] = (float4v){0.f, 0.f, 0.f, 0.f};
 #pragma unroll
                 for (int hs = 0; hs < 2; ++hs) {
                     const char* base = acquire();
@@ -467,7 +504,13 @@
                         *reinterpret_cast<uint4*>(dst + 8) = pack8(o + 8);
                     }
                 }
-            } else {
+            };
+            auto v_group = [&](int grp) {
+                float4v a1[4][TM];
+#pragma unroll
+                for (int t = 0; t < 4; ++t)
+#pragma unroll
+                    for (int mt = 0; mt < TM; ++mt) a1[t][mt] = (float4v){0.f, 0.f, 0.f, 0.f};
 #pragma unroll
                 for (int hs = 0; hs < 2; ++hs) {
                     const char* base = acquire();
@@ -496,7 +539,54 @@
                         }
                     }
                 }
-            }
+            };
+            auto prefetch_x = [&](auto part_c) {
+                constexpr int part = decltype(part_c)::value;
+                static_assert((NS - 2) * DPS + PFB[part + 1] - PFB[part] <= 63, "vmcnt field");
+                if constexpr (PREFETCH && PFB[part + 1] > PFB[part]) {
+                    if (has_next && p.do_post) {
+#pragma unroll
+                        for (int mt = 0; mt < TM; ++mt) {
+                            const int m = m0 + (int)gridDim.x * 128 + 16 * mt + fr;
+                            const int mm = m < p.M ? m : p.M - 1;
+                            const int seq = mm / p.Lout;
+                            const float* src = p.x + ((long)seq * p.seq_rows + p.row_off + (mm - seq * p.Lout)) * D + 4 * fq;
+#pragma unroll
+                            for (int t = 0; t < NT; ++t)
+                                if (mt * NT + t >= PFB[part] && mt * NT + t < PFB[part + 1])
+                                    acc[t][mt] = *reinterpret_cast<const float4v*>(src + 16 * t);
+                        }
+                        burst = part;
+                        boost = NS - 2;
+                        pref = true;
+                    }
+                }
+            };
+            if constexpr (!PREFETCH) {
+                for (int grp = 0; grp < n_groups; ++grp) {
+                    if (grp < n_qk) qk_group(grp);
+                    else v_group(grp);
+                }
+            } else {
+                constexpr int n_v2 = n_qk + (n_groups - n_qk) / 2;
+                prefetch_x(std::integral_constant<int, 0>{});
+                for (int grp = 0; grp < D / 64; ++grp) qk_group(grp);
+                prefetch_x(std::integral_constant<int, 1>{});
+                for (int grp = D / 64; grp < n_qk; ++grp) qk_group(grp);
+                prefetch_x(std::integral_constant<int, 2>{});
+                for (int grp = n_qk; grp < n_v2; ++grp) v_group(grp);
+                prefetch_x(std::integral_constant<int, 3>{});
+                for (int grp = n_v2; grp < n_groups; ++grp) v_group(grp);
+            }
+        }
+        if constexpr (PREFETCH) {
+            if (!pref) {
+#pragma unroll
+                for (int mt = 0; mt < TM; ++mt)
+#pragma unroll
+                    for (int t = 0; t < NT; ++t) asm volatile("" : "=v"(acc[t][mt]));
+            }
+            have_x = pref;
         }
     }
     asm volatile("s_waitcnt vmcnt(0)" ::: "memory");
@@ -578,7 +668,7 @@
     return off;
 }
 
-int fused_panel_launch(const PanelParams& p, int D, bool gated, hipStream_t st) {
+int fused_panel_launch(const PanelParams& p, int D, bool gated, hipStream_t st, int panel_grid) {
     SVC_REQUIRE(D == 384 || D == 512, "fused panel kernel: D must be 384 or 512");
     SVC_REQUIRE(p.M > 0 && p.Lout > 0 && p.I % 32 == 0, "fused panel kernel: shape");
     SVC_REQUIRE(!p.do_qkv || (p.M % 4 == 0 && p.Lout % 4 == 0 && p.row_off % 4 == 0), "fused panel kernel: v^T stores need 4-row groups");
@@ -593,7 +683,10 @@
     }
     const long want = (p.do_post ? slots_post(D, p.I) : 0) + (p.do_skip ? slots_skip(D) : 0) + (p.do_qkv ? slots_qkv(D) : 0);
     SVC_REQUIRE(want == p.n_slots, "fused panel kernel: slot count does not match the enabled phases");
-    const int grid = cdiv(p.M, 128);
+    SVC_REQUIRE(p.n_slots >= PG<384>::NS, "fused panel kernel: stream shorter than the weight ring");
+    const int n_panels = cdiv(p.M, 128);
+    const int cap = panel_grid < 0 ? n_panels : (panel_grid > 0 ? panel_grid : (ds->n_cus > 0 ? ds->n_cus : n_panels));
+    const int grid = n_panels < cap ? n_panels : cap;
     const bool prof = prof_enabled();
     if (prof) prof_begin(PROF_FUSED, st);
     static const int tm_env = [] { const char* e = getenv("SVC_FUSED_TM"); return e ? atoi(e) : 0; }();
```
